# joshua16266261/self-play-ai

Hardware: NVIDIA B200
Metric: MCTS simulations/sec (whole box) Connect4 @800 sims/move (higher is better)
Workload: dtype bf16

## Files before the change

self-play-ai_b200/csrc/evaluator_umma.cu:

```cuda
#include <cuda_bf16.h>

#include <cstring>
#include <mutex>

#include "evaluator_umma.cuh"
#include "umma_ptx.cuh"

namespace spb {
namespace umma {

template <class G>
struct Geo {
  static constexpr int W8 = (G::COLS == 7) ? 8 : 4;
  static constexpr int RP = G::ROWS + 1;
  static constexpr int BS = W8 * RP;
  static constexpr int NT = 4;
  static constexpr int NB = (NT * 128) / BS;
  static constexpr int LEAD = 16;
  static constexpr int Q = LEAD + NT * 128 + 16;
  static constexpr int P = G::ROWS * G::COLS;
  static constexpr int APAD = (G::A <= 8) ? 8 : 16;
};

constexpr int N_LAYERS = 10;
constexpr int HEAD_N = 48;
constexpr int SLOT_BYTES = 8192;
constexpr int N_SLOTS = 9;

__host__ __device__ constexpr int layer_n(int l) { return l == 9 ? HEAD_N : 64; }
__host__ __device__ constexpr int layer_kchunks(int l) { return l == 0 ? 2 : 8; }
__host__ __device__ constexpr int layer_tap_bytes(int l) { return layer_kchunks(l) * layer_n(l) * 16; }
__host__ __device__ constexpr size_t layer_offset(int l) {
  return l == 0 ? 0 : (size_t)9 * 2048 + (size_t)(l - 1) * 9 * SLOT_BYTES;
}
constexpr size_t OFF_BIAS = (size_t)9 * 2048 + (size_t)8 * 9 * SLOT_BYTES + (size_t)9 * 6144;
constexpr size_t OFF_WP = OFF_BIAS + (size_t)N_LAYERS * 64 * 4;
template <class G> __host__ __device__ constexpr size_t off_wv() { return OFF_WP + (size_t)G::A * Geo<G>::P * 32 * 4; }
template <class G> __host__ __device__ constexpr size_t off_fcb() { return off_wv<G>() + (size_t)Geo<G>::P * 8 * 4; }
template <class G> __host__ __device__ constexpr size_t image_bytes() { return off_fcb<G>() + 32 * 4; }

static inline uint16_t f2bf(float f) {
  uint32_t u;
  std::memcpy(&u, &f, 4);
  if ((u & 0x7F800000u) == 0x7F800000u) return (uint16_t)(u >> 16);
  u += 0x7FFFu + ((u >> 16) & 1u);
  return (uint16_t)(u >> 16);
}

template <class G>
static void pack_t(const HostNet& net, std::vector<uint8_t>* out) {
  using Ge = Geo<G>;
  out->assign(image_bytes<G>(), 0);
  uint8_t* img = out->data();
  for (int tap = 0; tap < 9; ++tap) {
    const HostNet::Conv& cv = net.conv[0];
    uint16_t* blk = reinterpret_cast<uint16_t*>(img + layer_offset(0) + (size_t)tap * layer_tap_bytes(0));
    for (int n = 0; n < 64; ++n)
      for (int k = 0; k < 16 && k < cv.ic; ++k)
        blk[((size_t)(k / 8) * 64 + n) * 8 + (k % 8)] = f2bf(cv.w[((size_t)n * cv.ic + k) * 9 + tap]);
  }
  for (int l = 1; l < N_LAYERS; ++l) {
    const int N = layer_n(l), KC = layer_kchunks(l);
    const int n_real = l == 9 ? NET_POLICY_CH + NET_VALUE_CH : 64;
    for (int ky = 0; ky < 3; ++ky) {
      uint16_t* blk = reinterpret_cast<uint16_t*>(img + layer_offset(l) + (size_t)ky * 3 * layer_tap_bytes(l));
      for (int n = 0; n < n_real; ++n) {
        const HostNet::Conv& cv = l < 9 ? net.conv[l] : (n < NET_POLICY_CH ? net.conv[9] : net.conv[10]);
        const int oc = (l == 9 && n >= NET_POLICY_CH) ? n - NET_POLICY_CH : n;
        for (int k = 0; k < KC * 8 && k < cv.ic; ++k) {
          const float* w9 = &cv.w[((size_t)oc * cv.ic + k) * 9 + ky * 3];
          uint16_t* row = blk + ((size_t)(k / 8) * 3 * N) * 8 + (k % 8);
          row[(size_t)n * 8] = f2bf(w9[1]);
          row[(size_t)(N + n) * 8] = f2bf(w9[2]);
          row[(size_t)(2 * N + n) * 8] = f2bf(w9[0]);
        }
      }
    }
  }
  float* bias = reinterpret_cast<float*>(img + OFF_BIAS);
  for (int l = 0; l < 9; ++l)
    for (int n = 0; n < 64; ++n) bias[l * 64 + n] = net.conv[l].b[n];
  for (int n = 0; n < NET_POLICY_CH; ++n) bias[9 * 64 + n] = net.conv[9].b[n];
  for (int n = 0; n < NET_VALUE_CH; ++n) bias[9 * 64 + NET_POLICY_CH + n] = net.conv[10].b[n];
  float* wp = reinterpret_cast<float*>(img + OFF_WP);
  for (int a = 0; a < G::A; ++a)
    for (int pos = 0; pos < Ge::P; ++pos)
      for (int ch = 0; ch < NET_POLICY_CH; ++ch)
        wp[((size_t)a * Ge::P + pos) * NET_POLICY_CH + ch] = net.pfc_w[(size_t)a * NET_POLICY_CH * Ge::P + (size_t)ch * Ge::P + pos];
  float* wv = reinterpret_cast<float*>(img + off_wv<G>());
  for (int pos = 0; pos < Ge::P; ++pos)
    for (int ch = 0; ch < NET_VALUE_CH; ++ch) wv[pos * 8 + ch] = net.vfc_w[(size_t)ch * Ge::P + pos];
  float* fcb = reinterpret_cast<float*>(img + off_fcb<G>());
  for (int a = 0; a < G::A; ++a) fcb[a] = net.pfc_b[a];
  fcb[16] = net.vfc_b[0];
}

void pack_weights(const HostNet& net, std::vector<uint8_t>* out) {
  if (net.game == SPB_GAME_CONNECT4) pack_t<Connect4>(net, out);
  else pack_t<TicTacToe>(net, out);
}

template <int W8, int Q, int KSTEPS, int NP>
__device__ __forceinline__ void issue_tile_triple(bool issuer, uint32_t a_lo_tile, uint32_t b_lo_base, uint32_t d_tmem,
                                                  bool first_tile, bool last_tile, uint32_t w_par, uint32_t bar_base,
                                                  uint32_t mid_bar, uint32_t mid_par) {
  constexpr uint32_t DESC_HI = (128u >> 4) | (1u << 14);
  constexpr uint32_t IDESC = make_idesc(NP);
#pragma unroll
  for (int ky = 0; ky < 3; ++ky) {
    const int shift = (ky - 1) * W8;
    if (ky == 2 && mid_bar) {
      mbar_wait(mid_bar, mid_par);
      tc_fence_after();
    }
    if (first_tile) {
      mbar_wait(bar_base + (uint32_t)ky * 8u, w_par);
      tc_fence_after();
    }
    if (issuer) {
#pragma unroll
      for (int kk = 0; kk < KSTEPS; ++kk) {
        const uint32_t a_lo = a_lo_tile + (uint32_t)(shift + kk * 2 * Q);
        const uint32_t b_lo = (b_lo_base + (uint32_t)(3 * ky) * (SLOT_BYTES >> 4) + (uint32_t)(kk * 2 * NP)) | ((uint32_t)NP << 16);
        umma_f16(d_tmem, ((uint64_t)DESC_HI << 32) | a_lo, ((uint64_t)DESC_HI << 32) | b_lo, IDESC, (ky | kk) != 0);
      }
      if (last_tile) umma_commit(bar_base + (uint32_t)(N_SLOTS + ky) * 8u);
    }
    __syncwarp();
  }
}

template <int W8, int Q>
__device__ __forceinline__ void issue_tile_stem(bool issuer, uint32_t a_lo_tile, uint32_t b_lo_base, uint32_t d_tmem, bool first_tile,
                                                bool last_tile, uint32_t w_par, uint32_t bar_base) {
  constexpr uint32_t DESC_HI = (128u >> 4) | (1u << 14);
  constexpr uint32_t IDESC = make_idesc(64);
#pragma unroll
  for (int ky = 0; ky < 3; ++ky) {
    if (first_tile) {
      mbar_wait(bar_base + (uint32_t)ky * 8u, w_par);
      tc_fence_after();
    }
    if (issuer) {
#pragma unroll
      for (int kx = 0; kx < 3; ++kx) {
        const uint32_t a_lo = a_lo_tile + (uint32_t)((ky - 1) * W8 + (kx - 1));
        const uint32_t b_lo = (b_lo_base + (uint32_t)(3 * ky) * (SLOT_BYTES >> 4) + (uint32_t)kx * (2048u >> 4)) | (64u << 16);
        umma_f16(d_tmem, ((uint64_t)DESC_HI << 32) | a_lo, ((uint64_t)DESC_HI << 32) | b_lo, IDESC, (ky | kx) != 0);
      }
      if (last_tile) umma_commit(bar_base + (uint32_t)(N_SLOTS + ky) * 8u);
    }
    __syncwarp();
  }
}

template <class G>
struct Smem {
  using Ge = Geo<G>;
  static constexpr int ACT_BYTES = 8 * Ge::Q * 16;
  static constexpr int OFF_ACT0 = 0;
  static constexpr int OFF_ACT1 = ACT_BYTES;
  static constexpr int OFF_W = 2 * ACT_BYTES;
  static constexpr int OFF_BIAS = OFF_W + N_SLOTS * SLOT_BYTES;
  static constexpr int OFF_LOGITS = OFF_BIAS + (N_LAYERS * 64 + 32) * 4;
  static constexpr int OFF_PART = OFF_LOGITS + Ge::NB * 16 * 4;
  static constexpr int OFF_STATES = OFF_PART + 8 * Ge::NB * 8 * 4;
  static constexpr int OFF_SLOTS = OFF_STATES + 2 * Ge::NB * 16;
  static constexpr int OFF_BARS = (OFF_SLOTS + 2 * Ge::NB * 4 + 15) & ~15;
  static constexpr int N_BARS = 2 * N_SLOTS + 4 + 2 * Ge::NT + 1 + 3 + 2;
  static constexpr int OFF_TMEM = OFF_BARS + N_BARS * 8;
  static constexpr int OFF_NB = OFF_TMEM + 16;
  static constexpr int TOTAL = OFF_NB + 32;
};
static_assert(Geo<Connect4>::NB <= 32 && Geo<TicTacToe>::NB <= 32, "one stager lane / one publishing lane per board");

static_assert(Smem<Connect4>::TOTAL <= 232448 && Smem<TicTacToe>::TOTAL <= 232448, "shared memory plan exceeds 227 KB");
constexpr int PRODUCER_WARP = 0, MMA_WARP = 1, STAGER_WARP = 2, SPARE_WARP = 3;
constexpr int EPI_WARP0 = 4, N_EPI_WARPS = 8;
constexpr int THREADS = 32 * (EPI_WARP0 + N_EPI_WARPS);
template <class G> struct RingCfg { static constexpr int TREE_WARPS = 4, REGS_LAUNCH = 128, REGS_LIGHT = 72, REGS_TREE = 96, REGS_EPILOGUE = 168; };
template <class G> constexpr int threads_ring() { return THREADS + 32 * RingCfg<G>::TREE_WARPS; }
template <class G> constexpr bool ring_budget_ok() {
  return 128 * RingCfg<G>::REGS_LIGHT + 256 * RingCfg<G>::REGS_EPILOGUE + 32 * RingCfg<G>::TREE_WARPS * RingCfg<G>::REGS_TREE <= threads_ring<G>() * RingCfg<G>::REGS_LAUNCH &&
         threads_ring<G>() * RingCfg<G>::REGS_LAUNCH <= 65536;
}
static_assert(ring_budget_ok<Connect4>() && ring_budget_ok<TicTacToe>(), "setmaxnreg budget exceeds the CTA's launch allocation");
constexpr uint32_t CLAIM_GRACE_NS = 4000;

struct EvalWork {
  const PState* states;
  const uint32_t* list;
  const uint32_t* count_dev;
  uint32_t max_n;
  float* out;
  int stride;
  float* logits_out;
};

#ifdef SPB_TRACE
__device__ unsigned long long g_trace[4][512];
#define TRACE_B0 (RING ? 300u : 0u)
#define TRACE(k, b, l, t) do { if (blockIdx.x == 0 && (b) >= TRACE_B0 && (b) < TRACE_B0 + 12u) g_trace[k][((((b) - TRACE_B0) * 10 + (l)) * 4 + (t))] = clock64(); } while (0)
__device__ unsigned long long g_trace_stager[16][4];
__device__ unsigned long long g_eval_times[64][4];
__device__ unsigned int g_eval_idx = 0;
__device__ __forceinline__ unsigned long long gtimer() { unsigned long long t; asm volatile("mov.u64 %0, %%globaltimer;" : "=l"(t)); return t; }
#define TRACE_ST(b, i) do { if (blockIdx.x == 0 && lane == 0 && (b) >= TRACE_B0 && (b) < TRACE_B0 + 12u) g_trace_stager[(b) - TRACE_B0][i] = clock64(); } while (0)
#define TRACE2(i) do { if (blockIdx.x == 0 && bb == TRACE_B0 && lane == 0) g_trace[3][480 + (warp == EPI_WARP0 ? 0 : 8) + (i)] = clock64(); } while (0)
#define TRACE3(i) do { if (blockIdx.x == 0 && bb == TRACE_B0 + 2u && l == 4 && t == 1 && lane == 0 && (warp == EPI_WARP0 || warp == EPI_WARP0 + 4)) g_trace[3][496 + (warp == EPI_WARP0 ? 0 : 8) + (i)] = clock64(); } while (0)
#else
#define TRACE3(i) ((void)0)
#define TRACE2(i) ((void)0)
#define TRACE(k, b, l, t) ((void)0)
#define TRACE_ST(b, i) ((void)0)
#endif

template <class G, bool RING>
__global__ void __launch_bounds__(RING ? threads_ring<G>() : THREADS, 1)
k_eval_umma(const uint8_t* __restrict__ image, const EvalWork W, const Trees T, const AsyncCtl C) {
  using Ge = Geo<G>;
  using Sm = Smem<G>;
  extern __shared__ __align__(1024) uint8_t smem[];
  const PState* __restrict__ states = RING ? T.leaf_state : W.states;
  const uint32_t* __restrict__ list = W.list;
  float* __restrict__ out = RING ? T.eval_out : W.out;
  const int stride = RING ? G::EVAL_STRIDE : W.stride;
  float* __restrict__ logits_out = RING ? nullptr : W.logits_out;
#ifdef SPB_TRACE
  const unsigned long long tr_entry = gtimer();
#endif
  asm volatile("griddepcontrol.launch_dependents;");
  const int tid = threadIdx.x, warp = tid >> 5, lane = tid & 31;
  const uint32_t s_base = smem_u32(smem);
  const uint32_t bar_base = s_base + Sm::OFF_BARS;
  auto bar_w_full = [&](int s) { return bar_base + (uint32_t)s * 8u; };
  auto bar_w_empty = [&](int s) { return bar_base + (uint32_t)(N_SLOTS + s) * 8u; };
  constexpr uint32_t BAR0 = 2 * N_SLOTS;
  auto bar_acc_full = [&](uint32_t set) { return bar_base + (BAR0 + set) * 8u; };
  auto bar_acc_drained = [&](uint32_t set) { return bar_base + (BAR0 + 2u + set) * 8u; };
  auto bar_act_ready = [&](int t) { return bar_base + (BAR0 + 4u + (uint32_t)t) * 8u; };
  auto bar_stage_ready = [&](int t) { return bar_base + (BAR0 + 4u + (uint32_t)Ge::NT + (uint32_t)t) * 8u; };
  const uint32_t bar_act0_free = bar_base + (BAR0 + 4u + 2u * (uint32_t)Ge::NT) * 8u;
  auto bar_batch = [&](uint32_t bb) { return bar_base + (BAR0 + 5u + 2u * (uint32_t)Ge::NT + (bb & 1u)) * 8u; };
  const uint32_t bar_claim_go = bar_base + (BAR0 + 7u + 2u * (uint32_t)Ge::NT) * 8u;
  const uint32_t bar_out_ready = bar_base + (BAR0 + 8u + 2u * (uint32_t)Ge::NT) * 8u;
  const uint32_t bar_out_free = bar_base + (BAR0 + 9u + 2u * (uint32_t)Ge::NT) * 8u;
  uint32_t* tmem_slot = reinterpret_cast<uint32_t*>(smem + Sm::OFF_TMEM);
  volatile uint32_t* s_nb = reinterpret_cast<volatile uint32_t*>(smem + Sm::OFF_NB);

  {
    uint4 z = make_uint4(0, 0, 0, 0);
    uint4* p = reinterpret_cast<uint4*>(smem);
    for (int i = tid; i < 2 * Sm::ACT_BYTES / 16; i += (int)blockDim.x) p[i] = z;
    const float* gb = reinterpret_cast<const float*>(image + OFF_BIAS);
    float* sb = reinterpret_cast<float*>(smem + Sm::OFF_BIAS);
    for (int i = tid; i < N_LAYERS * 64; i += (int)blockDim.x) sb[i] = gb[i];
    if (tid < 32) sb[N_LAYERS * 64 + tid] = reinterpret_cast<const float*>(image + off_fcb<G>())[tid];
  }
  if (tid == 0) {
    for (int s = 0; s < N_SLOTS; ++s) { mbar_init(bar_w_full(s), 1); mbar_init(bar_w_empty(s), 1); }
    for (uint32_t set = 0; set < 2; ++set) { mbar_init(bar_acc_full(set), 1); mbar_init(bar_acc_drained(set), N_EPI_WARPS); }
    for (int t = 0; t < Ge::NT; ++t) { mbar_init(bar_act_ready(t), N_EPI_WARPS); mbar_init(bar_stage_ready(t), 32); }
    mbar_init(bar_act0_free, 1);
    mbar_init(bar_batch(0), 1); mbar_init(bar_batch(1), 1); mbar_init(bar_claim_go, 1);
    mbar_init(bar_out_ready, 1); mbar_init(bar_out_free, 1);
    asm volatile("fence.mbarrier_init.release.cluster;" ::: "memory");
  }
  if (warp == MMA_WARP) tmem_alloc(smem_u32(tmem_slot), 512);
  fence_async_smem();
  tc_fence_before();
  __syncthreads();
  tc_fence_after();
  const uint32_t tmem_base = *tmem_slot;

  asm volatile("griddepcontrol.wait;" ::: "memory");
#ifdef SPB_TRACE
  const unsigned long long tr_wait = gtimer();
#endif
  const uint32_t n_total = RING ? 0u : min(__ldcg(W.count_dev), W.max_n);
  const uint32_t cta = blockIdx.x, ncta = gridDim.x;
  const uint32_t my_begin = (uint32_t)(((uint64_t)n_total * cta) / ncta);
  const uint32_t my_end = (uint32_t)(((uint64_t)n_total * (cta + 1)) / ncta);
  auto wait_batch = [&](uint32_t bb) -> uint32_t {
    mbar_wait(bar_batch(bb), (bb >> 1) & 1u);
    return s_nb[bb & 3u];
  };

#define SPB_REGS_LIGHT() do { if (RING) asm volatile("setmaxnreg.dec.sync.aligned.u32 %0;" ::"n"(RingCfg<G>::REGS_LIGHT)); } while (0)
#define SPB_REGS_TREE() do { if (RING) asm volatile("setmaxnreg.dec.sync.aligned.u32 %0;" ::"n"(RingCfg<G>::REGS_TREE)); } while (0)
#define SPB_REGS_EPILOGUE() do { if (RING) asm volatile("setmaxnreg.inc.sync.aligned.u32 %0;" ::"n"(RingCfg<G>::REGS_EPILOGUE)); } while (0)

  if (warp == PRODUCER_WARP) {
    SPB_REGS_LIGHT();
    if (lane == 0) {
      uint32_t use = 0;
      for (uint32_t b = 0; wait_batch(b) != 0u; ++b) {
        for (int l = 0; l < N_LAYERS; ++l) {
          const uint32_t bytes = (uint32_t)layer_tap_bytes(l);
          const uint8_t* src = image + layer_offset(l);
          for (int g = 0; g < 3; ++g) {
            if (use > 0) mbar_wait(bar_w_empty(g), (use - 1) & 1u);
            mbar_expect_tx(bar_w_full(g), 3 * bytes);
            bulk_g2s(s_base + Sm::OFF_W + (uint32_t)(3 * g) * SLOT_BYTES, src + (size_t)(3 * g) * bytes, 3 * bytes, bar_w_full(g));
          }
          ++use;
        }
      }
    }
  } else if (warp == MMA_WARP) {
    SPB_REGS_LIGHT();
    {
      const bool issuer = elect_one();
      const uint32_t b_lo_base = ((s_base + Sm::OFF_W) >> 4);
      uint32_t use = 0;
      uint32_t act_par = 0;
      uint32_t stage_par = 0;
      uint32_t g = 0;
      for (uint32_t b = 0;; ++b) {
        const uint32_t nb = wait_batch(b);
        if (nb == 0u) break;
        const int nt = (int)((nb * Ge::BS + 127) / 128);
        for (int l = 0; l < N_LAYERS; ++l) {
          if (RING && l == 7 && issuer) mbar_arrive(bar_claim_go);
          const uint32_t in_buf = s_base + ((l == 0 || (l >= 2 && (l & 1) == 0)) ? Sm::OFF_ACT0 : Sm::OFF_ACT1);
          const uint32_t a_lo_base = ((in_buf >> 4) + Ge::LEAD) | ((uint32_t)Ge::Q << 16);
          const uint32_t cur_par = (l == 0) ? stage_par : act_par;
          if (l == 0) stage_par ^= (1u << nt) - 1u; else act_par ^= (1u << nt) - 1u;
          for (int t = 0; t < nt; ++t, ++g) {
            uint32_t mid_bar = 0, mid_par = 0;
            if (l == 0) {
              const int wt = min(t + 1, nt - 1);
              mbar_wait(bar_stage_ready(wt), (cur_par >> wt) & 1u);
            } else {
              if (t == 0) mbar_wait(bar_act_ready(0), cur_par & 1u);
              if (t + 1 < nt) { mid_bar = bar_act_ready(t + 1); mid_par = (cur_par >> (t + 1)) & 1u; }
            }
            const uint32_t set = g & 1u, u = g >> 1;
            if (u > 0u) mbar_wait(bar_acc_drained(set), (u - 1u) & 1u);
            tc_fence_after();
            if (lane == 0) TRACE(0, b, l, t);
            const uint32_t a_lo_tile = a_lo_base + (uint32_t)t * 128u;
            const uint32_t d_tmem = tmem_base + set * 256u;
            const bool first = (t == 0), last = (t == nt - 1);
            if (l == 0)
              issue_tile_stem<Ge::W8, Ge::Q>(issuer, a_lo_tile, b_lo_base, d_tmem, first, last, use & 1u, bar_base);
            else if (l < 9)
              issue_tile_triple<Ge::W8, Ge::Q, 4, 192>(issuer, a_lo_tile, b_lo_base, d_tmem, first, last, use & 1u, bar_base, mid_bar, mid_par);
            else
              issue_tile_triple<Ge::W8, Ge::Q, 4, 3 * HEAD_N>(issuer, a_lo_tile, b_lo_base, d_tmem, first, last, use & 1u, bar_base, mid_bar, mid_par);
            if (issuer) {
              umma_commit(bar_acc_full(set));
              if (l == 8 && last) umma_commit(bar_act0_free);
            }
            __syncwarp();
            if (lane == 0) TRACE(1, b, l, t);
          }
          ++use;
        }
      }
    }
  } else if (warp == STAGER_WARP) {
    SPB_REGS_LIGHT();
    PState* s_states = reinterpret_cast<PState*>(smem + Sm::OFF_STATES);
    uint32_t* s_slots = reinterpret_cast<uint32_t*>(smem + Sm::OFF_SLOTS);
    Spin sp;
    if (RING) sp.init(C, *C.n_active);
    unsigned long long st_batches = 0, st_boards = 0, st_wait = 0;
    LeafClaimer lc;
    for (uint32_t bb = 0;; ++bb) {
      uint32_t nb = 0;
      PState st_mine = PState{};
      uint32_t slot_mine = 0;
      if (RING) {
        if (bb > 0) mbar_wait_backoff<64>(bar_claim_go, (bb - 1) & 1u);
        const unsigned long long tw0 = gtime_ns();
        TRACE_ST(bb, 0);
        nb = claim_batch(C, lc, ncta, (uint32_t)Ge::NB, CLAIM_GRACE_NS, sp, lane, &slot_mine);
        if (nb) { st_wait += gtime_ns() - tw0; ++st_batches; st_boards += nb; }
        TRACE_ST(bb, 1);
      } else {
        const uint32_t b0 = my_begin + bb * Ge::NB;
        nb = b0 < my_end ? min((uint32_t)Ge::NB, my_end - b0) : 0u;
        if ((uint32_t)lane < nb) slot_mine = list ? __ldcg(list + b0 + lane) : (b0 + lane);
      }
      if (lane == 0) {
        s_nb[bb & 3u] = nb;
        mbar_arrive(bar_batch(bb));
      }
      if (nb == 0u) {
        if (RING && lane == 0) {
          atomicAdd(&C.stats[ASTAT_BATCHES], st_batches);
          atomicAdd(&C.stats[ASTAT_BOARDS], st_boards);
          atomicAdd(&C.stats[ASTAT_CLAIM_WAIT_NS], st_wait);
          atomicAdd(&C.stats[ASTAT_EVAL_CTAS], 1ull);
        }
        break;
      }
      const int nt = (int)((nb * Ge::BS + 127) / 128);
      if ((uint32_t)lane < nb) {
        const ulonglong2 raw = __ldcg(reinterpret_cast<const ulonglong2*>(states + slot_mine));
        st_mine.x = raw.x; st_mine.o = raw.y;
      }
      if (bb > 0) mbar_wait_backoff<64>(bar_act0_free, (bb - 1) & 1u);
      TRACE_ST(bb, 2);
      PState* st_buf = s_states + (bb & 1u) * Ge::NB;
      if ((uint32_t)lane < nb) { s_slots[(bb & 1u) * Ge::NB + lane] = slot_mine; st_buf[lane] = st_mine; }
      __syncwarp();
      for (int t = 0; t < nt; ++t) {
#pragma unroll
        for (int q = 0; q < 4; ++q) {
          const int m = t * 128 + q * 32 + lane;
          const int bi = m / Ge::BS, rem = m % Ge::BS, r = rem / Ge::W8, c = rem % Ge::W8;
          uint4 v0 = make_uint4(0, 0, 0, 0);
          if ((uint32_t)bi < nb && r < G::ROWS && c < G::COLS) {
            const PState st = st_buf[bi];
            const float e0 = G::encode_cell(st, 0, r, c), e1 = G::encode_cell(st, 1, r, c), e2 = G::encode_cell(st, 2, r, c);
            v0.x = pack_bf16x2(e0, e1);
            v0.y = pack_bf16x2(e2, 0.0f);
          }
          *reinterpret_cast<uint4*>(smem + Sm::OFF_ACT0 + (size_t)(Ge::LEAD + m) * 16) = v0;
          *reinterpret_cast<uint4*>(smem + Sm::OFF_ACT0 + (size_t)Ge::Q * 16 + (size_t)(Ge::LEAD + m) * 16) = make_uint4(0, 0, 0, 0);
        }
        fence_async_smem();
        mbar_arrive(bar_stage_ready(t));
      }
      TRACE_ST(bb, 3);
    }
  } else if (warp >= EPI_WARP0 && warp < EPI_WARP0 + N_EPI_WARPS) {
    SPB_REGS_EPILOGUE();
    const int et = tid - 32 * EPI_WARP0;
    const int quad = warp & 3;
    const int half = (warp - EPI_WARP0) >> 2;
    const int row_in_tile = quad * 32 + lane;
    const float* s_bias = reinterpret_cast<const float*>(smem + Sm::OFF_BIAS);
    float* s_logits = reinterpret_cast<float*>(smem + Sm::OFF_LOGITS);
    uint32_t* s_slots = reinterpret_cast<uint32_t*>(smem + Sm::OFF_SLOTS);
    const float* g_wp = reinterpret_cast<const float*>(image + OFF_WP);
    const float* g_wv = reinterpret_cast<const float*>(image + off_wv<G>());
    uint32_t eg = 0;

    auto conv_epilogue = [&](uint32_t bb, int l, int t_begin = 0, int t_end = Ge::NT) {
      const uint32_t nb = s_nb[bb & 3u];
      const int nt = min((int)((nb * Ge::BS + 127) / 128), t_end);
      const bool in0 = (l == 0 || (l >= 2 && (l & 1) == 0));
      uint8_t* dst_buf = smem + (in0 ? Sm::OFF_ACT1 : Sm::OFF_ACT0);
      const bool has_skip = (l >= 2 && (l & 1) == 0);
      const bool stash_skip = (l & 1) == 0 && l <= 6;
      float bias_r[32];
#pragma unroll
      for (int q = 0; q < 8; ++q) {
        const float4 bv = *reinterpret_cast<const float4*>(s_bias + l * 64 + half * 32 + q * 4);
        bias_r[4 * q] = bv.x; bias_r[4 * q + 1] = bv.y; bias_r[4 * q + 2] = bv.z; bias_r[4 * q + 3] = bv.w;
      }
      for (int t = t_begin; t < nt; ++t, ++eg) {
        const int m = t * 128 + row_in_tile;
        const int bi = m / Ge::BS, rem = m % Ge::BS, r = rem / Ge::W8, c = rem % Ge::W8;
        const bool valid = (uint32_t)bi < nb && r < G::ROWS && c < G::COLS;
        uint8_t* drow = dst_buf + (size_t)(half * 4) * Ge::Q * 16 + (size_t)(Ge::LEAD + m) * 16;
        const uint32_t set = eg & 1u;
        TRACE3(0);
        mbar_wait(bar_acc_full(set), (eg >> 1) & 1u);
        tc_fence_after();
        if (et == 0) TRACE(2, bb, l, t);
        TRACE3(1);
        const uint32_t taddr = tmem_base + ((uint32_t)(quad * 32) << 16) + set * 256u + (uint32_t)half * 32u;
        uint32_t a[32], e[32], f[32];
        tmem_ld16(taddr, a);
        tmem_ld16(taddr + 16u, a + 16);
        if (l != 0) {
          tmem_ld16(taddr + 64u, e);
          tmem_ld16(taddr + 80u, e + 16);
          tmem_ld16(taddr + 128u, f);
          tmem_ld16(taddr + 144u, f + 16);
        }
        tmem_ld_wait();
        tc_fence_before();
        __syncwarp();
        if (lane == 0) mbar_arrive(bar_acc_drained(set));
        TRACE3(2);
        float v[32];
#pragma unroll
        for (int q = 0; q < 32; q += 2) {
          if (l == 0) { v[q] = __uint_as_float(a[q]); v[q + 1] = __uint_as_float(a[q + 1]); continue; }
          const float e0 = __uint_as_float(__shfl_down_sync(0xffffffffu, e[q], 1)), e1 = __uint_as_float(__shfl_down_sync(0xffffffffu, e[q + 1], 1));
          const float f0 = __uint_as_float(__shfl_up_sync(0xffffffffu, f[q], 1)), f1 = __uint_as_float(__shfl_up_sync(0xffffffffu, f[q + 1], 1));
          v[q] = __uint_as_float(a[q]); v[q + 1] = __uint_as_float(a[q + 1]);
          add2(v[q], v[q + 1], e0, e1);
          if (lane != 0) add2(v[q], v[q + 1], f0, f1);
        }
        TRACE3(3);
        const uint32_t skaddr = tmem_base + ((uint32_t)(quad * 32) << 16) + ((t & 1) ? 448u : 192u) + (uint32_t)(t >> 1) * 32u + (uint32_t)half * 16u;
        uint32_t sk[16];
        if (has_skip) tmem_ld16(skaddr, sk);
#pragma unroll
        for (int q = 0; q < 32; q += 2) add2(v[q], v[q + 1], bias_r[q], bias_r[q + 1]);
        if (has_skip) {
          tmem_ld_wait();
#pragma unroll
          for (int q = 0; q < 16; ++q) add2(v[2 * q], v[2 * q + 1], bf_lo(sk[q]), bf_hi(sk[q]));
        }
        uint32_t o[16];
#pragma unroll
        for (int q = 0; q < 16; ++q) o[q] = valid ? pack_relu_bf16x2(v[2 * q], v[2 * q + 1]) : 0u;
#pragma unroll
        for (int j = 0; j < 4; ++j)
          *reinterpret_cast<uint4*>(drow + (size_t)j * Ge::Q * 16) = make_uint4(o[4 * j], o[4 * j + 1], o[4 * j + 2], o[4 * j + 3]);
        if (stash_skip) { tmem_st16(skaddr, o); tmem_st_wait(); }
        TRACE3(4);
        fence_async_smem();
        __syncwarp();
        if (lane == 0) mbar_arrive(bar_act_ready(t));
        TRACE3(5);
        if (et == 0) TRACE(3, bb, l, t);
      }
    };

    auto head_epilogue = [&](uint32_t bb) {
      const uint32_t nb = s_nb[bb & 3u];
      const int nt = (int)((nb * Ge::BS + 127) / 128);
      const float* bias = s_bias + 9 * 64;
      for (int t = 0; t < nt; ++t, ++eg) {
        const int m = t * 128 + row_in_tile;
        const int bi = m / Ge::BS, rem = m % Ge::BS, r = rem / Ge::W8, c = rem % Ge::W8;
        const bool valid = (uint32_t)bi < nb && r < G::ROWS && c < G::COLS;
        const uint32_t set = eg & 1u;
        mbar_wait(bar_acc_full(set), (eg >> 1) & 1u);
        tc_fence_after();
        if (et == 0) TRACE(2, bb, 9, t);
        const uint32_t taddr = tmem_base + ((uint32_t)(quad * 32) << 16) + set * 256u;
        uint32_t a[16], av[4], e[16], ev[4], f[16], fv[4];
        tmem_ld16(taddr + (uint32_t)half * 16u, a);
        tmem_ld16(taddr + (uint32_t)HEAD_N + (uint32_t)half * 16u, e);
        tmem_ld16(taddr + 2u * (uint32_t)HEAD_N + (uint32_t)half * 16u, f);
        if (half == 1) { tmem_ld4(taddr + 32u, av); tmem_ld4(taddr + (uint32_t)HEAD_N + 32u, ev); tmem_ld4(taddr + 2u * (uint32_t)HEAD_N + 32u, fv); }
        tmem_ld_wait();
        tc_fence_before();
        __syncwarp();
        if (lane == 0) mbar_arrive(bar_acc_drained(set));
#pragma unroll
        for (int q = 0; q < 16; ++q) {
          const float e1 = __uint_as_float(__shfl_down_sync(0xffffffffu, e[q], 1));
          const float f1 = __uint_as_float(__shfl_up_sync(0xffffffffu, f[q], 1));
          float v = __uint_as_float(a[q]) + e1;
          if (lane != 0) v += f1;
          a[q] = __float_as_uint(v);
        }
        if (half == 1) {
#pragma unroll
          for (int q = 0; q < 3; ++q) {
            const float e1 = __uint_as_float(__shfl_down_sync(0xffffffffu, ev[q], 1));
            const float f1 = __uint_as_float(__shfl_up_sync(0xffffffffu, fv[q], 1));
            av[q] = __float_as_uint((__uint_as_float(av[q]) + e1) + (lane == 0 ? 0.0f : f1));
          }
        }
        if (valid) {
          uint8_t* prow = smem + Sm::OFF_ACT0 + (size_t)(Ge::LEAD + m) * 16;
#pragma unroll
          for (int j = 0; j < 2; ++j) {
            uint4 o;
            const float* bj = bias + half * 16 + j * 8;
            o.x = pack_bf16x2(fmaxf(__uint_as_float(a[j * 8 + 0]) + bj[0], 0.f), fmaxf(__uint_as_float(a[j * 8 + 1]) + bj[1], 0.f));
            o.y = pack_bf16x2(fmaxf(__uint_as_float(a[j * 8 + 2]) + bj[2], 0.f), fmaxf(__uint_as_float(a[j * 8 + 3]) + bj[3], 0.f));
            o.z = pack_bf16x2(fmaxf(__uint_as_float(a[j * 8 + 4]) + bj[4], 0.f), fmaxf(__uint_as_float(a[j * 8 + 5]) + bj[5], 0.f));
            o.w = pack_bf16x2(fmaxf(__uint_as_float(a[j * 8 + 6]) + bj[6], 0.f), fmaxf(__uint_as_float(a[j * 8 + 7]) + bj[7], 0.f));
            *reinterpret_cast<uint4*>(prow + (size_t)(2 + half * 2 + j) * Ge::Q * 16) = o;
          }
          if (half == 1) {
            uint4 o = make_uint4(0, 0, 0, 0);
            o.x = pack_bf16x2(fmaxf(__uint_as_float(av[0]) + bias[32], 0.f), fmaxf(__uint_as_float(av[1]) + bias[33], 0.f));
            o.y = pack_bf16x2(fmaxf(__uint_as_float(av[2]) + bias[34], 0.f), 0.f);
            *reinterpret_cast<uint4*>(prow + (size_t)6 * Ge::Q * 16) = o;
          }
        }
        if (et == 0) TRACE(3, bb, 9, t);
      }
    };

    constexpr int LH_P = Ge::P;
    constexpr int NOUT = G::A + 1;
    const bool is_pol = et < 4 * LH_P, is_val = !is_pol && et < 5 * LH_P;
    const int pos = is_pol ? (et % LH_P) : (is_val ? et - 4 * LH_P : 0);
    const int c4 = is_pol ? (et / LH_P) : 4;
    auto load_head_weights = [&](float (&w)[8][8], int og) {
#pragma unroll
      for (int s = 0; s < 8; ++s) {
        const int o = og + s;
#pragma unroll
        for (int j = 0; j < 8; ++j) w[s][j] = 0.0f;
        const float* src = nullptr;
        if (is_pol && o < G::A) src = g_wp + ((size_t)o * LH_P + pos) * NET_POLICY_CH + c4 * 8;
        if (is_val && o == G::A) src = g_wv + pos * 8;
        if (src) {
          const float4 w0 = __ldg(reinterpret_cast<const float4*>(src)), w1 = __ldg(reinterpret_cast<const float4*>(src) + 1);
          w[s][0] = w0.x; w[s][1] = w0.y; w[s][2] = w0.z; w[s][3] = w0.w;
          w[s][4] = w1.x; w[s][5] = w1.y; w[s][6] = w1.z; w[s][7] = w1.w;
        }
      }
    };
    auto heads_partials = [&](uint32_t bb, float (&w)[8][8], uint32_t bi_begin = 0, uint32_t bi_end = Ge::NB) {
      const uint32_t nb = s_nb[bb & 3u];
      const uint32_t bend = min(nb, bi_end);
      float* s_part = reinterpret_cast<float*>(smem + Sm::OFF_PART);
      const int we = warp - EPI_WARP0;
      const uint32_t roff = (uint32_t)((is_pol || is_val ? (2 + c4) * Ge::Q * 16 : 0) + ((pos / G::COLS) * Ge::W8 + (pos % G::COLS)) * 16);
      TRACE2(0);
      {
        TRACE2(1);
        const bool b4 = lane & 16, b3 = lane & 8, b2 = lane & 4;
        uint4 vn[3];
#pragma unroll
        for (int k = 0; k < 3; ++k)
          vn[k] = *reinterpret_cast<const uint4*>(smem + Sm::OFF_ACT0 + (size_t)(Ge::LEAD + min(bi_begin + (uint32_t)k, nb - 1u) * Ge::BS) * 16 + roff);
        for (uint32_t bi0 = bi_begin; bi0 < bend; bi0 += 3) {
          float sres[3];
          uint4 v[3];
#pragma unroll
          for (int k = 0; k < 3; ++k) {
            v[k] = vn[k];
            vn[k] = *reinterpret_cast<const uint4*>(smem + Sm::OFF_ACT0 + (size_t)(Ge::LEAD + min(bi0 + 3u + (uint32_t)k, nb - 1u) * Ge::BS) * 16 + roff);
          }
          float q[3][4], r2[3][2];
#pragma unroll
          for (int k = 0; k < 3; ++k) {
            const float x0 = bf_lo(v[k].x), x1 = bf_hi(v[k].x), x2 = bf_lo(v[k].y), x3 = bf_hi(v[k].y);
            const float x4 = bf_lo(v[k].z), x5 = bf_hi(v[k].z), x6 = bf_lo(v[k].w), x7 = bf_hi(v[k].w);
            float p[8];
#pragma unroll
            for (int s = 0; s < 8; ++s) {
              float a = x0 * w[s][0];
              a = fmaf(x1, w[s][1], a); a = fmaf(x2, w[s][2], a); a = fmaf(x3, w[s][3], a);
              a = fmaf(x4, w[s][4], a); a = fmaf(x5, w[s][5], a); a = fmaf(x6, w[s][6], a); a = fmaf(x7, w[s][7], a);
              p[s] = a;
            }
#pragma unroll
            for (int i = 0; i < 4; ++i) q[k][i] = (b4 ? p[i + 4] : p[i]) + __shfl_xor_sync(0xffffffffu, b4 ? p[i] : p[i + 4], 16);
          }
#pragma unroll
          for (int k = 0; k < 3; ++k) {
#pragma unroll
            for (int i = 0; i < 2; ++i) r2[k][i] = (b3 ? q[k][i + 2] : q[k][i]) + __shfl_xor_sync(0xffffffffu, b3 ? q[k][i] : q[k][i + 2], 8);
          }
#pragma unroll
          for (int k = 0; k < 3; ++k) sres[k] = (b2 ? r2[k][1] : r2[k][0]) + __shfl_xor_sync(0xffffffffu, b2 ? r2[k][0] : r2[k][1], 4);
#pragma unroll
          for (int k = 0; k < 3; ++k) sres[k] += __shfl_xor_sync(0xffffffffu, sres[k], 2);
#pragma unroll
          for (int k = 0; k < 3; ++k) sres[k] += __shfl_xor_sync(0xffffffffu, sres[k], 1);
          if ((lane & 3) == 0) {
#pragma unroll
            for (int k = 0; k < 3; ++k)
              if (bi0 + (uint32_t)k < nb) s_part[((size_t)we * Ge::NB + bi0 + k) * 8 + (lane >> 2)] = sres[k];
          }
        }
        TRACE2(2);
      }
    };
    auto heads_reduce = [&](uint32_t bb, int og) {
      const uint32_t nb = s_nb[bb & 3u];
      const float* s_part = reinterpret_cast<const float*>(smem + Sm::OFF_PART);
      epi_bar_sync();
      if (og == 0 && bb > 0) mbar_wait(bar_out_free, (bb - 1) & 1u);
      for (int i = et; i < (int)nb * 8; i += 256) {
        const int bi = i >> 3, sl = i & 7, o = og + sl;
        if (o < NOUT) {
          float acc = 0.0f;
#pragma unroll
          for (int wv_ = 0; wv_ < 8; ++wv_) acc += s_part[((size_t)wv_ * Ge::NB + bi) * 8 + sl];
          s_logits[bi * 16 + (o == G::A ? 15 : o)] = acc;
        }
      }
      epi_bar_sync();
      TRACE2(3);
    };
    auto heads_softmax = [&](uint32_t bb) {
      const uint32_t nb = s_nb[bb & 3u];
      constexpr int LG = G::A <= 7 ? 8 : 16;
      const float* fcb = s_bias + N_LAYERS * 64;
      const int a = et % LG;
      for (uint32_t bi = (uint32_t)(et / LG); bi < ((nb + 256 / LG - 1) / (256 / LG)) * (256 / LG); bi += 256 / LG) {
        const bool live = bi < nb;
        const float raw = live ? s_logits[bi * 16 + (a == LG - 1 ? 15 : a)] : 0.0f;
        const float lg = (a < G::A) ? raw + fcb[a] : -INFINITY;
        float mx = lg;
#pragma unroll
        for (int o = LG / 2; o >= 1; o >>= 1) mx = fmaxf(mx, __shfl_xor_sync(0xffffffffu, mx, o));
        const float ex = (a < G::A) ? expf(lg - mx) : 0.0f;
        float sum = 0.0f;
#pragma unroll
        for (int k = 0; k < G::A; ++k) sum += __shfl_sync(0xffffffffu, ex, (lane & ~(LG - 1)) + k);
        if (live) {
          if (a < G::A) s_logits[bi * 16 + a] = ex / sum;
          else if (a == LG - 1) s_logits[bi * 16 + 15] = tanhf(raw + fcb[16]);
          if (logits_out && a < G::A) logits_out[(size_t)s_slots[(bb & 1u) * Ge::NB + bi] * G::A + a] = lg;
        }
      }
      TRACE2(4);
      epi_bar_sync();
      if (et == 0) mbar_arrive(bar_out_ready);
      TRACE2(5);
    };
    auto linear_heads = [&](uint32_t bb, float (&w_first)[8][8]) {
      heads_partials(bb, w_first);
      heads_reduce(bb, 0);
      for (int og = 8; og < NOUT; og += 8) {
        float w[8][8];
        load_head_weights(w, og);
        heads_partials(bb, w);
        heads_reduce(bb, og);
      }
      heads_softmax(bb);
    };

    constexpr uint32_t NOT_YET = 0xFFFFFFFFu;
    uint32_t nb_cur = wait_batch(0);
    if (nb_cur != 0u) conv_epilogue(0, 0);
    bool l1_done = false;
    for (uint32_t b = 0; nb_cur != 0u; ++b) {
      for (int l = l1_done ? 2 : 1; l < 9; ++l) conv_epilogue(b, l);
      l1_done = false;
      head_epilogue(b);
      if (et == 0) s_nb[4] = mbar_test(bar_batch(b + 1), ((b + 1) >> 1) & 1u) ? s_nb[(b + 1) & 3u] : NOT_YET;
      epi_bar_sync();
      uint32_t nb_next = s_nb[4];
      float w_heads[8][8];
      if (nb_next != NOT_YET) {
        load_head_weights(w_heads, 0);
        if (nb_next != 0u) conv_epilogue(b + 1, 0);
        if (NOUT <= 8 && nb_next != 0u) {
          heads_partials(b, w_heads);
          epi_bar_sync();
          conv_epilogue(b + 1, 1);
          l1_done = true;
          heads_reduce(b, 0);
          heads_softmax(b);
        } else {
          linear_heads(b, w_heads);
        }
      } else {
        load_head_weights(w_heads, 0);
        linear_heads(b, w_heads);
        nb_next = wait_batch(b + 1);
        if (nb_next != 0u) conv_epilogue(b + 1, 0);
      }
      nb_cur = nb_next;
    }
  }

  if (RING && warp >= EPI_WARP0 + N_EPI_WARPS) {
    SPB_REGS_TREE();
    tree_worker<G>(T, C, lane);
  } else if (warp == SPARE_WARP) {
    SPB_REGS_LIGHT();
    const float* s_logits = reinterpret_cast<const float*>(smem + Sm::OFF_LOGITS);
    const uint32_t* s_slots = reinterpret_cast<const uint32_t*>(smem + Sm::OFF_SLOTS);
    for (uint32_t b = 0;; ++b) {
      const uint32_t nb = wait_batch(b);
      if (nb == 0u) break;
      mbar_wait(bar_out_ready, b & 1u);
      uint32_t slot = 0;
      float rec[G::A + 1];
      if ((uint32_t)lane < nb) {
        slot = s_slots[(b & 1u) * Ge::NB + lane];
#pragma unroll
        for (int a = 0; a < G::A; ++a) rec[a] = s_logits[lane * 16 + a];
        rec[G::A] = s_logits[lane * 16 + 15];
      }
      __syncwarp();
      if (lane == 0) mbar_arrive(bar_out_free);
      if ((uint32_t)lane < nb) {
        float* o = out + (size_t)slot * stride;
#pragma unroll
        for (int a = 0; a <= G::A; ++a) o[a] = rec[a];
      }
      if (RING) ring_push_warp(C.ready, nb, slot, lane);
    }
  }

  tc_fence_before();
  __syncthreads();
  if (warp == MMA_WARP) { tc_fence_after(); tmem_dealloc(tmem_base, 512); }
#ifdef SPB_TRACE
  if (blockIdx.x == 0 && tid == 0) {
    const unsigned int i = g_eval_idx++ & 63u;
    g_eval_times[i][0] = tr_entry; g_eval_times[i][1] = tr_wait; g_eval_times[i][2] = gtimer();
  }
#endif
}

template <class G, bool RING>
static cudaError_t prepare(int* sm_count_out) {
  static std::mutex mu;
  static int sm_counts[64] = {};
  int dev = 0;
  cudaError_t e = cudaGetDevice(&dev);
  if (e != cudaSuccess) return e;
  if (dev < 0 || dev >= 64) return cudaErrorInvalidDevice;
  std::lock_guard<std::mutex> lock(mu);
  if (sm_counts[dev] == 0) {
    int n = 0;
    e = cudaDeviceGetAttribute(&n, cudaDevAttrMultiProcessorCount, dev);
    if (e == cudaSuccess) e = cudaFuncSetAttribute(k_eval_umma<G, RING>, cudaFuncAttributeMaxDynamicSharedMemorySize, Smem<G>::TOTAL);
    if (e != cudaSuccess) return e;
    sm_counts[dev] = n;
  }
  *sm_count_out = sm_counts[dev];
  return cudaSuccess;
}

template <class G>
static cudaError_t launch_t(const Evaluator::DevNet& net, const PState* states, const uint32_t* list, const uint32_t* count_dev,
                            uint32_t max_n, float* out, int stride, float* logits_out, cudaStream_t stream, bool overlap) {
  int sm_count = 0;
  cudaError_t e = prepare<G, false>(&sm_count);
  if (e != cudaSuccess) return e;
  const unsigned grid = (unsigned)std::max(1, std::min<int>(sm_count, (int)max_n));
  cudaLaunchConfig_t cfg = {};
  cfg.gridDim = dim3(grid);
  cfg.blockDim = dim3(THREADS);
  cfg.dynamicSmemBytes = Smem<G>::TOTAL;
  cfg.stream = stream;
  cudaLaunchAttribute attr[1];
  attr[0].id = cudaLaunchAttributeProgrammaticStreamSerialization;
  attr[0].val.programmaticStreamSerializationAllowed = overlap ? 1 : 0;
  cfg.attrs = attr;
  cfg.numAttrs = 1;
  EvalWork W{states, list, count_dev, max_n, out, stride, logits_out};
  return cudaLaunchKernelEx(&cfg, k_eval_umma<G, false>, reinterpret_cast<const uint8_t*>(net.w_umma), W, Trees{}, AsyncCtl{});
}

template <class G>
static cudaError_t launch_ring_t(const Evaluator::DevNet& net, const Trees& T, const AsyncCtl& C, cudaStream_t stream) {
  int sm_count = 0;
  cudaError_t e = prepare<G, true>(&sm_count);
  if (e != cudaSuccess) return e;
  const unsigned grid = (unsigned)std::max(1, std::min<int>(sm_count, (int)T.G));
  k_eval_umma<G, true><<<grid, threads_ring<G>(), Smem<G>::TOTAL, stream>>>(reinterpret_cast<const uint8_t*>(net.w_umma), EvalWork{}, T, C);
  return cudaGetLastError();
}

#ifdef SPB_TRACE
extern "C" int spb_debug_eval_times_v2(unsigned long long* out) {
  unsigned int z = 0;
  int rc = (int)cudaMemcpyFromSymbol(out, g_eval_times, sizeof(unsigned long long) * 64 * 4);
  rc |= (int)cudaMemcpyToSymbol(g_eval_idx, &z, sizeof z);
  return rc;
}
extern "C" int spb_debug_trace_stager(unsigned long long* out) { return (int)cudaMemcpyFromSymbol(out, g_trace_stager, sizeof(unsigned long long) * 16 * 4); }
extern "C" int spb_debug_trace_v2(unsigned long long* out, int reset) {
  int rc = (int)cudaMemcpyFromSymbol(out, g_trace, sizeof(unsigned long long) * 4 * 512);
  if (reset) { static unsigned long long z[4 * 512]; rc |= (int)cudaMemcpyToSymbol(g_trace, z, sizeof z); }
  return rc;
}
#endif

cudaError_t launch(const Evaluator::DevNet& net, int game, const PState* states, const uint32_t* list, const uint32_t* count_dev,
                   uint32_t max_n, float* out, int stride, float* logits_out, cudaStream_t stream, bool overlap) {
  if (game == SPB_GAME_CONNECT4) return launch_t<Connect4>(net, states, list, count_dev, max_n, out, stride, logits_out, stream, overlap);
  return launch_t<TicTacToe>(net, states, list, count_dev, max_n, out, stride, logits_out, stream, overlap);
}

cudaError_t launch_ring(const Evaluator::DevNet& net, int game, const Trees& T, const AsyncCtl& C, cudaStream_t stream) {
  if (game == SPB_GAME_CONNECT4) return launch_ring_t<Connect4>(net, T, C, stream);
  return launch_ring_t<TicTacToe>(net, T, C, stream);
}

}
}
```

self-play-ai_b200/csrc/umma_ptx.cuh:

```cuda
#pragma once
#include <cuda_bf16.h>
#include <cstdint>

namespace spb {
namespace umma {

__device__ __forceinline__ uint32_t smem_u32(const void* p) { return (uint32_t)__cvta_generic_to_shared(p); }
__device__ __forceinline__ void mbar_init(uint32_t bar, uint32_t count) { asm volatile("mbarrier.init.shared::cta.b64 [%0], %1;" ::"r"(bar), "r"(count)); }
__device__ __forceinline__ void mbar_wait(uint32_t bar, uint32_t parity) {
  uint32_t ok;
  do {
#ifdef SPB_MBAR_HINT
    asm volatile("{\n.reg .pred p;\nmbarrier.try_wait.parity.shared::cta.b64 p, [%1], %2, %3;\nselp.u32 %0, 1, 0, p;\n}"
                 : "=r"(ok) : "r"(bar), "r"(parity), "r"((uint32_t)SPB_MBAR_HINT) : "memory");
#else
    asm volatile("{\n.reg .pred p;\nmbarrier.try_wait.parity.shared::cta.b64 p, [%1], %2;\nselp.u32 %0, 1, 0, p;\n}"
                 : "=r"(ok) : "r"(bar), "r"(parity) : "memory");
#endif
  } while (!ok);
}
__device__ __forceinline__ void mbar_wait_sleep(uint32_t bar, uint32_t parity) {
  uint32_t ok;
  for (;;) {
    asm volatile("{\n.reg .pred p;\nmbarrier.try_wait.parity.shared::cta.b64 p, [%1], %2;\nselp.u32 %0, 1, 0, p;\n}"
                 : "=r"(ok) : "r"(bar), "r"(parity) : "memory");
    if (ok) break;
    __nanosleep(200);
  }
}
template <int NS>
__device__ __forceinline__ void mbar_wait_backoff(uint32_t bar, uint32_t parity) {
  uint32_t ok;
  for (;;) {
    asm volatile("{\n.reg .pred p;\nmbarrier.try_wait.parity.shared::cta.b64 p, [%1], %2;\nselp.u32 %0, 1, 0, p;\n}"
                 : "=r"(ok) : "r"(bar), "r"(parity) : "memory");
    if (ok) break;
    if (NS > 0) __nanosleep(NS);
  }
}
__device__ __forceinline__ bool mbar_test(uint32_t bar, uint32_t parity) {
  uint32_t ok;
  asm volatile("{\n.reg .pred p;\nmbarrier.test_wait.parity.shared::cta.b64 p, [%1], %2;\nselp.u32 %0, 1, 0, p;\n}"
               : "=r"(ok) : "r"(bar), "r"(parity) : "memory");
  return ok != 0;
}
__device__ __forceinline__ void mbar_arrive(uint32_t bar) { asm volatile("mbarrier.arrive.shared::cta.b64 _, [%0];" ::"r"(bar) : "memory"); }
__device__ __forceinline__ void mbar_expect_tx(uint32_t bar, uint32_t bytes) { asm volatile("mbarrier.arrive.expect_tx.shared::cta.b64 _, [%0], %1;" ::"r"(bar), "r"(bytes) : "memory"); }
__device__ __forceinline__ void bulk_g2s(uint32_t dst, const void* src, uint32_t bytes, uint32_t bar) {
  asm volatile("cp.async.bulk.shared::cluster.global.mbarrier::complete_tx::bytes [%0], [%1], %2, [%3];" ::"r"(dst), "l"(src), "r"(bytes), "r"(bar) : "memory");
}
__device__ __forceinline__ void tmem_alloc(uint32_t dst_smem, uint32_t ncols) {
  asm volatile("tcgen05.alloc.cta_group::1.sync.aligned.shared::cta.b32 [%0], %1;" ::"r"(dst_smem), "r"(ncols) : "memory");
  asm volatile("tcgen05.relinquish_alloc_permit.cta_group::1.sync.aligned;" ::: "memory");
}
__device__ __forceinline__ void tmem_dealloc(uint32_t taddr, uint32_t ncols) { asm volatile("tcgen05.dealloc.cta_group::1.sync.aligned.b32 %0, %1;" ::"r"(taddr), "r"(ncols) : "memory"); }
__device__ __forceinline__ void umma_f16(uint32_t d_tmem, uint64_t adesc, uint64_t bdesc, uint32_t idesc, uint32_t accumulate) {
  asm volatile("{\n.reg .pred p;\nsetp.ne.b32 p, %4, 0;\ntcgen05.mma.cta_group::1.kind::f16 [%0], %1, %2, %3, p;\n}"
               ::"r"(d_tmem), "l"(adesc), "l"(bdesc), "r"(idesc), "r"(accumulate) : "memory");
}
__device__ __forceinline__ void umma_commit(uint32_t bar) { asm volatile("tcgen05.commit.cta_group::1.mbarrier::arrive::one.shared::cluster.b64 [%0];" ::"r"(bar) : "memory"); }
__device__ __forceinline__ void tc_fence_before() { asm volatile("tcgen05.fence::before_thread_sync;" ::: "memory"); }
__device__ __forceinline__ void tc_fence_after() { asm volatile("tcgen05.fence::after_thread_sync;" ::: "memory"); }
__device__ __forceinline__ void fence_async_smem() { asm volatile("fence.proxy.async.shared::cta;" ::: "memory"); }
__device__ __forceinline__ bool elect_one() {
  uint32_t pred;
  asm volatile("{\n.reg .pred P1;\nelect.sync _|P1, 0xffffffff;\nselp.u32 %0, 1, 0, P1;\n}" : "=r"(pred));
  return pred != 0;
}
__device__ __forceinline__ void epi_bar_sync() { asm volatile("bar.sync 1, 256;" ::: "memory"); }

__device__ __forceinline__ void tmem_ld16(uint32_t taddr, uint32_t* r) {
  asm volatile("tcgen05.ld.sync.aligned.32x32b.x16.b32 {%0,%1,%2,%3,%4,%5,%6,%7,%8,%9,%10,%11,%12,%13,%14,%15}, [%16];"
               : "=r"(r[0]), "=r"(r[1]), "=r"(r[2]), "=r"(r[3]), "=r"(r[4]), "=r"(r[5]), "=r"(r[6]), "=r"(r[7]), "=r"(r[8]), "=r"(r[9]),
                 "=r"(r[10]), "=r"(r[11]), "=r"(r[12]), "=r"(r[13]), "=r"(r[14]), "=r"(r[15])
               : "r"(taddr));
}
__device__ __forceinline__ void tmem_ld4(uint32_t taddr, uint32_t* r) {
  asm volatile("tcgen05.ld.sync.aligned.32x32b.x4.b32 {%0,%1,%2,%3}, [%4];" : "=r"(r[0]), "=r"(r[1]), "=r"(r[2]), "=r"(r[3]) : "r"(taddr));
}
__device__ __forceinline__ void tmem_st16(uint32_t taddr, const uint32_t* r) {
  asm volatile("tcgen05.st.sync.aligned.32x32b.x16.b32 [%0], {%1,%2,%3,%4,%5,%6,%7,%8,%9,%10,%11,%12,%13,%14,%15,%16};"
               ::"r"(taddr), "r"(r[0]), "r"(r[1]), "r"(r[2]), "r"(r[3]), "r"(r[4]), "r"(r[5]), "r"(r[6]), "r"(r[7]), "r"(r[8]), "r"(r[9]),
                 "r"(r[10]), "r"(r[11]), "r"(r[12]), "r"(r[13]), "r"(r[14]), "r"(r[15]) : "memory");
}
__device__ __forceinline__ void tmem_st_wait() { asm volatile("tcgen05.wait::st.sync.aligned;" ::: "memory"); }
__device__ __forceinline__ void tmem_ld_wait() { asm volatile("tcgen05.wait::ld.sync.aligned;" ::: "memory"); }

__device__ __forceinline__ uint64_t make_desc(uint32_t addr, uint32_t lbo, uint32_t sbo) {
  return (uint64_t)((addr >> 4) & 0x3FFFu) | ((uint64_t)((lbo >> 4) & 0x3FFFu) << 16) | ((uint64_t)((sbo >> 4) & 0x3FFFu) << 32) |
         ((uint64_t)1 << 46);
}
__host__ __device__ constexpr uint32_t make_idesc(int N) {
  return (1u << 4) | (1u << 7) | (1u << 10) | ((uint32_t)(N >> 3) << 17) | ((uint32_t)(128 >> 4) << 24);
}

__device__ __forceinline__ uint32_t pack_bf16x2(float lo, float hi) {
  __nv_bfloat162 v = __floats2bfloat162_rn(lo, hi);
  return *reinterpret_cast<uint32_t*>(&v);
}
__device__ __forceinline__ void add2(float& x0, float& x1, float y0, float y1) {
  uint64_t x, y;
  asm("mov.b64 %0, {%1, %2};" : "=l"(x) : "f"(x0), "f"(x1));
  asm("mov.b64 %0, {%1, %2};" : "=l"(y) : "f"(y0), "f"(y1));
  asm("add.rn.f32x2 %0, %0, %1;" : "+l"(x) : "l"(y));
  asm("mov.b64 {%0, %1}, %2;" : "=f"(x0), "=f"(x1) : "l"(x));
}
__device__ __forceinline__ uint32_t pack_relu_bf16x2(float lo, float hi) {
  uint32_t d;
  asm("cvt.rn.relu.bf16x2.f32 %0, %1, %2;" : "=r"(d) : "f"(hi), "f"(lo));
  return d;
}
__device__ __forceinline__ float bf_lo(uint32_t u) { return __uint_as_float(u << 16); }
__device__ __forceinline__ float bf_hi(uint32_t u) { return __uint_as_float(u & 0xFFFF0000u); }

}
}
```

Before: 45.82 million.

## Fuse policy/value FC into head epilogue with per-tile partial sums

The head conv epilogue now computes the policy and value linear layers directly from its TMEM accumulators. Each thread applies register-held or shared-memory-staged weights and reduces partials with warp shuffles into a per-board shared buffer. The spare warp finishes the cross-group sum, softmax and tanh, which removes the activation write-back to shared memory, the separate partials, reduce and softmax phases, and several named barriers. The head layer also uses smaller tiles aligned to whole boards, and the MMA warp waits only on the activation tiles each head tile needs. This costs more registers in the epilogue warps, extra shared memory for the weights, and the overlap of the head with the next batch's early layers is dropped.

Result: no change. 45.72 million (median of 6 runs) (-0.2%).

```diff
diff --git a/self-play-ai_b200/csrc/evaluator_umma.cu b/self-play-ai_b200/csrc/evaluator_umma.cu
--- a/self-play-ai_b200/csrc/evaluator_umma.cu
+++ b/self-play-ai_b200/csrc/evaluator_umma.cu
@@ -19,7 +19,9 @@
   static constexpr int LEAD = 16;
   static constexpr int Q = LEAD + NT * 128 + 16;
   static constexpr int P = G::ROWS * G::COLS;
-  static constexpr int APAD = (G::A <= 8) ? 8 : 16;
+  static constexpr int HB = 128 / BS;
+  static constexpr int HS = HB * BS;
+  static constexpr int HG = BS / 8;
 };
 
 constexpr int N_LAYERS = 10;
@@ -86,7 +88,7 @@
   for (int a = 0; a < G::A; ++a)
     for (int pos = 0; pos < Ge::P; ++pos)
       for (int ch = 0; ch < NET_POLICY_CH; ++ch)
-        wp[((size_t)a * Ge::P + pos) * NET_POLICY_CH + ch] = net.pfc_w[(size_t)a * NET_POLICY_CH * Ge::P + (size_t)ch * Ge::P + pos];
+        wp[(((size_t)a * 8 + ch / 4) * Ge::P + pos) * 4 + ch % 4] = net.pfc_w[(size_t)a * NET_POLICY_CH * Ge::P + (size_t)ch * Ge::P + pos];
   float* wv = reinterpret_cast<float*>(img + off_wv<G>());
   for (int pos = 0; pos < Ge::P; ++pos)
     for (int ch = 0; ch < NET_VALUE_CH; ++ch) wv[pos * 8 + ch] = net.vfc_w[(size_t)ch * Ge::P + pos];
@@ -152,6 +154,12 @@
     }
     __syncwarp();
   }
+}
+
+__device__ __forceinline__ float4 ldg_f4_here(const float* p) {
+  float4 v;
+  asm volatile("ld.global.nc.v4.f32 {%0,%1,%2,%3}, [%4];" : "=f"(v.x), "=f"(v.y), "=f"(v.z), "=f"(v.w) : "l"(p));
+  return v;
 }
 
 template <class G>
@@ -162,9 +170,13 @@
   static constexpr int OFF_ACT1 = ACT_BYTES;
   static constexpr int OFF_W = 2 * ACT_BYTES;
   static constexpr int OFF_BIAS = OFF_W + N_SLOTS * SLOT_BYTES;
-  static constexpr int OFF_LOGITS = OFF_BIAS + (N_LAYERS * 64 + 32) * 4;
-  static constexpr int OFF_PART = OFF_LOGITS + Ge::NB * 16 * 4;
-  static constexpr int OFF_STATES = OFF_PART + 8 * Ge::NB * 8 * 4;
+  static constexpr int OREG = G::A <= 7 ? 6 : 4;
+  static constexpr int NOUTP = (G::A + 1 + 7) & ~7;
+  static constexpr int OFF_WPS = OFF_BIAS + (N_LAYERS * 64 + 32) * 4;
+  static constexpr int OFF_WVS = OFF_WPS + (G::A - OREG) * 2 * 16 * Ge::P * 4;
+  static constexpr int OFF_HPART = OFF_WVS + Ge::P * 16;
+  static constexpr int HPART_BOARD = Ge::HG * 2 * NOUTP + 1;
+  static constexpr int OFF_STATES = (OFF_HPART + Ge::NB * HPART_BOARD * 4 + 15) & ~15;
   static constexpr int OFF_SLOTS = OFF_STATES + 2 * Ge::NB * 16;
   static constexpr int OFF_BARS = (OFF_SLOTS + 2 * Ge::NB * 4 + 15) & ~15;
   static constexpr int N_BARS = 2 * N_SLOTS + 4 + 2 * Ge::NT + 1 + 3 + 2;
@@ -198,19 +210,17 @@
 };
 
 #ifdef SPB_TRACE
-__device__ unsigned long long g_trace[4][512];
+__device__ unsigned long long g_trace[4][1024];
 #define TRACE_B0 (RING ? 300u : 0u)
-#define TRACE(k, b, l, t) do { if (blockIdx.x == 0 && (b) >= TRACE_B0 && (b) < TRACE_B0 + 12u) g_trace[k][((((b) - TRACE_B0) * 10 + (l)) * 4 + (t))] = clock64(); } while (0)
+#define TRACE(k, b, l, t) do { if (blockIdx.x == 0 && (b) >= TRACE_B0 && (b) < TRACE_B0 + 12u) g_trace[k][((((b) - TRACE_B0) * 10 + (l)) * 8 + (t))] = clock64(); } while (0)
 __device__ unsigned long long g_trace_stager[16][4];
 __device__ unsigned long long g_eval_times[64][4];
 __device__ unsigned int g_eval_idx = 0;
 __device__ __forceinline__ unsigned long long gtimer() { unsigned long long t; asm volatile("mov.u64 %0, %%globaltimer;" : "=l"(t)); return t; }
 #define TRACE_ST(b, i) do { if (blockIdx.x == 0 && lane == 0 && (b) >= TRACE_B0 && (b) < TRACE_B0 + 12u) g_trace_stager[(b) - TRACE_B0][i] = clock64(); } while (0)
-#define TRACE2(i) do { if (blockIdx.x == 0 && bb == TRACE_B0 && lane == 0) g_trace[3][480 + (warp == EPI_WARP0 ? 0 : 8) + (i)] = clock64(); } while (0)
-#define TRACE3(i) do { if (blockIdx.x == 0 && bb == TRACE_B0 + 2u && l == 4 && t == 1 && lane == 0 && (warp == EPI_WARP0 || warp == EPI_WARP0 + 4)) g_trace[3][496 + (warp == EPI_WARP0 ? 0 : 8) + (i)] = clock64(); } while (0)
+#define TRACE3(i) do { if (blockIdx.x == 0 && bb == TRACE_B0 + 2u && l == 4 && t == 1 && lane == 0 && (warp == EPI_WARP0 || warp == EPI_WARP0 + 4)) g_trace[3][992 + (warp == EPI_WARP0 ? 0 : 8) + (i)] = clock64(); } while (0)
 #else
 #define TRACE3(i) ((void)0)
-#define TRACE2(i) ((void)0)
 #define TRACE(k, b, l, t) ((void)0)
 #define TRACE_ST(b, i) ((void)0)
 #endif
@@ -256,6 +266,11 @@
     float* sb = reinterpret_cast<float*>(smem + Sm::OFF_BIAS);
     for (int i = tid; i < N_LAYERS * 64; i += (int)blockDim.x) sb[i] = gb[i];
     if (tid < 32) sb[N_LAYERS * 64 + tid] = reinterpret_cast<const float*>(image + off_fcb<G>())[tid];
+    const float4* gw = reinterpret_cast<const float4*>(image + OFF_WP) + Sm::OREG * 8 * Ge::P;
+    float4* sw = reinterpret_cast<float4*>(smem + Sm::OFF_WPS);
+    for (int i = tid; i < (G::A - Sm::OREG) * 8 * Ge::P; i += (int)blockDim.x) sw[i] = gw[i];
+    for (int i = tid; i < Ge::P; i += (int)blockDim.x)
+      reinterpret_cast<float4*>(smem + Sm::OFF_WVS)[i] = reinterpret_cast<const float4*>(image + off_wv<G>())[2 * i];
   }
   if (tid == 0) {
     for (int s = 0; s < N_SLOTS; ++s) { mbar_init(bar_w_full(s), 1); mbar_init(bar_w_empty(s), 1); }
@@ -263,7 +278,7 @@
     for (int t = 0; t < Ge::NT; ++t) { mbar_init(bar_act_ready(t), N_EPI_WARPS); mbar_init(bar_stage_ready(t), 32); }
     mbar_init(bar_act0_free, 1);
     mbar_init(bar_batch(0), 1); mbar_init(bar_batch(1), 1); mbar_init(bar_claim_go, 1);
-    mbar_init(bar_out_ready, 1); mbar_init(bar_out_free, 1);
+    mbar_init(bar_out_ready, N_EPI_WARPS); mbar_init(bar_out_free, 1);
     asm volatile("fence.mbarrier_init.release.cluster;" ::: "memory");
   }
   if (warp == MMA_WARP) tmem_alloc(smem_u32(tmem_slot), 512);
@@ -320,28 +335,32 @@
         const uint32_t nb = wait_batch(b);
         if (nb == 0u) break;
         const int nt = (int)((nb * Ge::BS + 127) / 128);
+        const int nht = (int)((nb + Ge::HB - 1) / Ge::HB);
         for (int l = 0; l < N_LAYERS; ++l) {
           if (RING && l == 7 && issuer) mbar_arrive(bar_claim_go);
           const uint32_t in_buf = s_base + ((l == 0 || (l >= 2 && (l & 1) == 0)) ? Sm::OFF_ACT0 : Sm::OFF_ACT1);
           const uint32_t a_lo_base = ((in_buf >> 4) + Ge::LEAD) | ((uint32_t)Ge::Q << 16);
           const uint32_t cur_par = (l == 0) ? stage_par : act_par;
           if (l == 0) stage_par ^= (1u << nt) - 1u; else act_par ^= (1u << nt) - 1u;
-          for (int t = 0; t < nt; ++t, ++g) {
+          const int ntl = l == 9 ? nht : nt, ts = l == 9 ? Ge::HS : 128;
+          int waited = 0;
+          for (int t = 0; t < ntl; ++t, ++g) {
             uint32_t mid_bar = 0, mid_par = 0;
             if (l == 0) {
               const int wt = min(t + 1, nt - 1);
               mbar_wait(bar_stage_ready(wt), (cur_par >> wt) & 1u);
             } else {
-              if (t == 0) mbar_wait(bar_act_ready(0), cur_par & 1u);
-              if (t + 1 < nt) { mid_bar = bar_act_ready(t + 1); mid_par = (cur_par >> (t + 1)) & 1u; }
+              const int need = min((ts * t + 127) / 128, nt - 1), need_mid = min((ts * t + 127 + Ge::W8) / 128, nt - 1);
+              for (; waited <= need; ++waited) mbar_wait(bar_act_ready(waited), (cur_par >> waited) & 1u);
+              if (need_mid >= waited) { mid_bar = bar_act_ready(need_mid); mid_par = (cur_par >> need_mid) & 1u; waited = need_mid + 1; }
             }
             const uint32_t set = g & 1u, u = g >> 1;
             if (u > 0u) mbar_wait(bar_acc_drained(set), (u - 1u) & 1u);
             tc_fence_after();
             if (lane == 0) TRACE(0, b, l, t);
-            const uint32_t a_lo_tile = a_lo_base + (uint32_t)t * 128u;
+            const uint32_t a_lo_tile = a_lo_base + (uint32_t)(t * ts);
             const uint32_t d_tmem = tmem_base + set * 256u;
-            const bool first = (t == 0), last = (t == nt - 1);
+            const bool first = (t == 0), last = (t == ntl - 1);
             if (l == 0)
               issue_tile_stem<Ge::W8, Ge::Q>(issuer, a_lo_tile, b_lo_base, d_tmem, first, last, use & 1u, bar_base);
             else if (l < 9)
@@ -433,10 +452,7 @@
     const int half = (warp - EPI_WARP0) >> 2;
     const int row_in_tile = quad * 32 + lane;
     const float* s_bias = reinterpret_cast<const float*>(smem + Sm::OFF_BIAS);
-    float* s_logits = reinterpret_cast<float*>(smem + Sm::OFF_LOGITS);
-    uint32_t* s_slots = reinterpret_cast<uint32_t*>(smem + Sm::OFF_SLOTS);
     const float* g_wp = reinterpret_cast<const float*>(image + OFF_WP);
-    const float* g_wv = reinterpret_cast<const float*>(image + off_wv<G>());
     uint32_t eg = 0;
 
     auto conv_epilogue = [&](uint32_t bb, int l, int t_begin = 0, int t_end = Ge::NT) {
@@ -516,242 +532,122 @@
     };
 
     auto head_epilogue = [&](uint32_t bb) {
+      constexpr int OREG = Sm::OREG, NOUTP = Sm::NOUTP;
       const uint32_t nb = s_nb[bb & 3u];
-      const int nt = (int)((nb * Ge::BS + 127) / 128);
+      const int nht = (int)((nb + Ge::HB - 1) / Ge::HB);
       const float* bias = s_bias + 9 * 64;
-      for (int t = 0; t < nt; ++t, ++eg) {
-        const int m = t * 128 + row_in_tile;
-        const int bi = m / Ge::BS, rem = m % Ge::BS, r = rem / Ge::W8, c = rem % Ge::W8;
-        const bool valid = (uint32_t)bi < nb && r < G::ROWS && c < G::COLS;
+      const int rem = row_in_tile % Ge::BS, r = rem / Ge::W8, c = rem % Ge::W8, grp = rem >> 3;
+      const bool cell = row_in_tile < Ge::HS && r < G::ROWS && c < G::COLS;
+      const int pos = cell ? r * G::COLS + c : 0;
+      float w[OREG][16];
+#pragma unroll
+      for (int o = 0; o < OREG; ++o) {
+#pragma unroll
+        for (int q = 0; q < 4; ++q) {
+          const float4 v = ldg_f4_here(g_wp + (((size_t)o * 8 + half * 4 + q) * Ge::P + pos) * 4);
+          w[o][4 * q] = v.x; w[o][4 * q + 1] = v.y; w[o][4 * q + 2] = v.z; w[o][4 * q + 3] = v.w;
+        }
+      }
+      const float4* s_wps = reinterpret_cast<const float4*>(smem + Sm::OFF_WPS) + half * 4 * Ge::P + pos;
+      float* s_hpart = reinterpret_cast<float*>(smem + Sm::OFF_HPART);
+      for (int t = 0; t < nht; ++t, ++eg) {
+        const uint32_t bi = (uint32_t)(t * Ge::HB + row_in_tile / Ge::BS);
+        const bool valid = cell && bi < nb;
         const uint32_t set = eg & 1u;
         mbar_wait(bar_acc_full(set), (eg >> 1) & 1u);
         tc_fence_after();
         if (et == 0) TRACE(2, bb, 9, t);
         const uint32_t taddr = tmem_base + ((uint32_t)(quad * 32) << 16) + set * 256u;
-        uint32_t a[16], av[4], e[16], ev[4], f[16], fv[4];
+        uint32_t a[16], av[4], e[16], ev[4];
         tmem_ld16(taddr + (uint32_t)half * 16u, a);
         tmem_ld16(taddr + (uint32_t)HEAD_N + (uint32_t)half * 16u, e);
-        tmem_ld16(taddr + 2u * (uint32_t)HEAD_N + (uint32_t)half * 16u, f);
-        if (half == 1) { tmem_ld4(taddr + 32u, av); tmem_ld4(taddr + (uint32_t)HEAD_N + 32u, ev); tmem_ld4(taddr + 2u * (uint32_t)HEAD_N + 32u, fv); }
+        tmem_ld4(taddr + 32u, av);
+        tmem_ld4(taddr + (uint32_t)HEAD_N + 32u, ev);
+        tmem_ld_wait();
+        float v[20];
+#pragma unroll
+        for (int q = 0; q < 16; q += 2) {
+          v[q] = __uint_as_float(a[q]); v[q + 1] = __uint_as_float(a[q + 1]);
+          add2(v[q], v[q + 1], __uint_as_float(__shfl_down_sync(0xffffffffu, e[q], 1)), __uint_as_float(__shfl_down_sync(0xffffffffu, e[q + 1], 1)));
+        }
+#pragma unroll
+        for (int q = 0; q < 4; q += 2) {
+          v[16 + q] = __uint_as_float(av[q]); v[17 + q] = __uint_as_float(av[q + 1]);
+          add2(v[16 + q], v[17 + q], __uint_as_float(__shfl_down_sync(0xffffffffu, ev[q], 1)), __uint_as_float(__shfl_down_sync(0xffffffffu, ev[q + 1], 1)));
+        }
+        tmem_ld16(taddr + 2u * (uint32_t)HEAD_N + (uint32_t)half * 16u, e);
+        tmem_ld4(taddr + 2u * (uint32_t)HEAD_N + 32u, ev);
         tmem_ld_wait();
         tc_fence_before();
         __syncwarp();
         if (lane == 0) mbar_arrive(bar_acc_drained(set));
-#pragma unroll
-        for (int q = 0; q < 16; ++q) {
-          const float e1 = __uint_as_float(__shfl_down_sync(0xffffffffu, e[q], 1));
-          const float f1 = __uint_as_float(__shfl_up_sync(0xffffffffu, f[q], 1));
-          float v = __uint_as_float(a[q]) + e1;
-          if (lane != 0) v += f1;
-          a[q] = __float_as_uint(v);
-        }
-        if (half == 1) {
-#pragma unroll
-          for (int q = 0; q < 3; ++q) {
-            const float e1 = __uint_as_float(__shfl_down_sync(0xffffffffu, ev[q], 1));
-            const float f1 = __uint_as_float(__shfl_up_sync(0xffffffffu, fv[q], 1));
-            av[q] = __float_as_uint((__uint_as_float(av[q]) + e1) + (lane == 0 ? 0.0f : f1));
+        if (t == 0 && bb > 0) mbar_wait(bar_out_free, (bb - 1) & 1u);
+        uint32_t xp[10];
+#pragma unroll
+        for (int q = 0; q < 20; q += 2) {
+          const uint32_t* fs = q < 16 ? e + q : ev + (q - 16);
+          const float f0 = __uint_as_float(__shfl_up_sync(0xffffffffu, fs[0], 1)), f1 = __uint_as_float(__shfl_up_sync(0xffffffffu, fs[1], 1));
+          if (lane != 0) add2(v[q], v[q + 1], f0, f1);
+          const float4 bq = *reinterpret_cast<const float4*>(bias + (q < 16 ? half * 16 + (q & ~3) : 32 + ((q - 16) & ~3)));
+          add2(v[q], v[q + 1], (q & 2) ? bq.z : bq.x, (q & 2) ? bq.w : bq.y);
+          xp[q / 2] = valid ? pack_relu_bf16x2(v[q], v[q + 1]) : 0u;
+        }
+        auto partial = [&](int o) -> float {
+          float s0 = 0.f, s1 = 0.f;
+          if (o < OREG) {
+#pragma unroll
+            for (int k = 0; k < 8; ++k) fma2(s0, s1, bf_lo(xp[k]), bf_hi(xp[k]), w[o][2 * k], w[o][2 * k + 1]);
+          } else if (o < G::A) {
+#pragma unroll
+            for (int q = 0; q < 4; ++q) {
+              const float4 wq = s_wps[((o - OREG) * 8 + q) * Ge::P];
+              fma2(s0, s1, bf_lo(xp[2 * q]), bf_hi(xp[2 * q]), wq.x, wq.y);
+              fma2(s0, s1, bf_lo(xp[2 * q + 1]), bf_hi(xp[2 * q + 1]), wq.z, wq.w);
+            }
+          } else if (o == G::A) {
+            const float4 wv = reinterpret_cast<const float4*>(smem + Sm::OFF_WVS)[pos];
+            fma2(s0, s1, bf_lo(xp[8]), bf_hi(xp[8]), half == 1 ? wv.x : 0.f, half == 1 ? wv.y : 0.f);
+            s0 = fmaf(bf_lo(xp[9]), half == 1 ? wv.z : 0.f, s0);
           }
-        }
-        if (valid) {
-          uint8_t* prow = smem + Sm::OFF_ACT0 + (size_t)(Ge::LEAD + m) * 16;
-#pragma unroll
-          for (int j = 0; j < 2; ++j) {
-            uint4 o;
-            const float* bj = bias + half * 16 + j * 8;
-            o.x = pack_bf16x2(fmaxf(__uint_as_float(a[j * 8 + 0]) + bj[0], 0.f), fmaxf(__uint_as_float(a[j * 8 + 1]) + bj[1], 0.f));
-            o.y = pack_bf16x2(fmaxf(__uint_as_float(a[j * 8 + 2]) + bj[2], 0.f), fmaxf(__uint_as_float(a[j * 8 + 3]) + bj[3], 0.f));
-            o.z = pack_bf16x2(fmaxf(__uint_as_float(a[j * 8 + 4]) + bj[4], 0.f), fmaxf(__uint_as_float(a[j * 8 + 5]) + bj[5], 0.f));
-            o.w = pack_bf16x2(fmaxf(__uint_as_float(a[j * 8 + 6]) + bj[6], 0.f), fmaxf(__uint_as_float(a[j * 8 + 7]) + bj[7], 0.f));
-            *reinterpret_cast<uint4*>(prow + (size_t)(2 + half * 2 + j) * Ge::Q * 16) = o;
-          }
-          if (half == 1) {
-            uint4 o = make_uint4(0, 0, 0, 0);
-            o.x = pack_bf16x2(fmaxf(__uint_as_float(av[0]) + bias[32], 0.f), fmaxf(__uint_as_float(av[1]) + bias[33], 0.f));
-            o.y = pack_bf16x2(fmaxf(__uint_as_float(av[2]) + bias[34], 0.f), 0.f);
-            *reinterpret_cast<uint4*>(prow + (size_t)6 * Ge::Q * 16) = o;
-          }
+          return s0 + s1;
+        };
+        const bool b2 = lane & 4, b1 = lane & 2, b0 = lane & 1;
+        const bool store = row_in_tile < Ge::HS && bi < nb;
+        float* dst = s_hpart + bi * Sm::HPART_BOARD + (grp * 2 + half) * NOUTP + (lane & 7);
+#pragma unroll
+        for (int k = 0; k < NOUTP / 8; ++k) {
+          float pk[8], q4[4], q2[2];
+#pragma unroll
+          for (int i = 0; i < 8; ++i) pk[i] = partial(8 * k + i);
+#pragma unroll
+          for (int i = 0; i < 4; ++i) q4[i] = (b2 ? pk[i + 4] : pk[i]) + __shfl_xor_sync(0xffffffffu, b2 ? pk[i] : pk[i + 4], 4);
+#pragma unroll
+          for (int i = 0; i < 2; ++i) q2[i] = (b1 ? q4[i + 2] : q4[i]) + __shfl_xor_sync(0xffffffffu, b1 ? q4[i] : q4[i + 2], 2);
+          const float sum = (b0 ? q2[1] : q2[0]) + __shfl_xor_sync(0xffffffffu, b0 ? q2[0] : q2[1], 1);
+          if (store) dst[8 * k] = sum;
         }
         if (et == 0) TRACE(3, bb, 9, t);
       }
+      __syncwarp();
+      if (lane == 0) mbar_arrive(bar_out_ready);
     };
 
-    constexpr int LH_P = Ge::P;
-    constexpr int NOUT = G::A + 1;
-    const bool is_pol = et < 4 * LH_P, is_val = !is_pol && et < 5 * LH_P;
-    const int pos = is_pol ? (et % LH_P) : (is_val ? et - 4 * LH_P : 0);
-    const int c4 = is_pol ? (et / LH_P) : 4;
-    auto load_head_weights = [&](float (&w)[8][8], int og) {
-#pragma unroll
-      for (int s = 0; s < 8; ++s) {
-        const int o = og + s;
-#pragma unroll
-        for (int j = 0; j < 8; ++j) w[s][j] = 0.0f;
-        const float* src = nullptr;
-        if (is_pol && o < G::A) src = g_wp + ((size_t)o * LH_P + pos) * NET_POLICY_CH + c4 * 8;
-        if (is_val && o == G::A) src = g_wv + pos * 8;
-        if (src) {
-          const float4 w0 = __ldg(reinterpret_cast<const float4*>(src)), w1 = __ldg(reinterpret_cast<const float4*>(src) + 1);
-          w[s][0] = w0.x; w[s][1] = w0.y; w[s][2] = w0.z; w[s][3] = w0.w;
-          w[s][4] = w1.x; w[s][5] = w1.y; w[s][6] = w1.z; w[s][7] = w1.w;
-        }
-      }
-    };
-    auto heads_partials = [&](uint32_t bb, float (&w)[8][8], uint32_t bi_begin = 0, uint32_t bi_end = Ge::NB) {
-      const uint32_t nb = s_nb[bb & 3u];
-      const uint32_t bend = min(nb, bi_end);
-      float* s_part = reinterpret_cast<float*>(smem + Sm::OFF_PART);
-      const int we = warp - EPI_WARP0;
-      const uint32_t roff = (uint32_t)((is_pol || is_val ? (2 + c4) * Ge::Q * 16 : 0) + ((pos / G::COLS) * Ge::W8 + (pos % G::COLS)) * 16);
-      TRACE2(0);
-      {
-        TRACE2(1);
-        const bool b4 = lane & 16, b3 = lane & 8, b2 = lane & 4;
-        uint4 vn[3];
-#pragma unroll
-        for (int k = 0; k < 3; ++k)
-          vn[k] = *reinterpret_cast<const uint4*>(smem + Sm::OFF_ACT0 + (size_t)(Ge::LEAD + min(bi_begin + (uint32_t)k, nb - 1u) * Ge::BS) * 16 + roff);
-        for (uint32_t bi0 = bi_begin; bi0 < bend; bi0 += 3) {
-          float sres[3];
-          uint4 v[3];
-#pragma unroll
-          for (int k = 0; k < 3; ++k) {
-            v[k] = vn[k];
-            vn[k] = *reinterpret_cast<const uint4*>(smem + Sm::OFF_ACT0 + (size_t)(Ge::LEAD + min(bi0 + 3u + (uint32_t)k, nb - 1u) * Ge::BS) * 16 + roff);
-          }
-          float q[3][4], r2[3][2];
-#pragma unroll
-          for (int k = 0; k < 3; ++k) {
-            const float x0 = bf_lo(v[k].x), x1 = bf_hi(v[k].x), x2 = bf_lo(v[k].y), x3 = bf_hi(v[k].y);
-            const float x4 = bf_lo(v[k].z), x5 = bf_hi(v[k].z), x6 = bf_lo(v[k].w), x7 = bf_hi(v[k].w);
-            float p[8];
-#pragma unroll
-            for (int s = 0; s < 8; ++s) {
-              float a = x0 * w[s][0];
-              a = fmaf(x1, w[s][1], a); a = fmaf(x2, w[s][2], a); a = fmaf(x3, w[s][3], a);
-              a = fmaf(x4, w[s][4], a); a = fmaf(x5, w[s][5], a); a = fmaf(x6, w[s][6], a); a = fmaf(x7, w[s][7], a);
-              p[s] = a;
-            }
-#pragma unroll
-            for (int i = 0; i < 4; ++i) q[k][i] = (b4 ? p[i + 4] : p[i]) + __shfl_xor_sync(0xffffffffu, b4 ? p[i] : p[i + 4], 16);
-          }
-#pragma unroll
-          for (int k = 0; k < 3; ++k) {
-#pragma unroll
-            for (int i = 0; i < 2; ++i) r2[k][i] = (b3 ? q[k][i + 2] : q[k][i]) + __shfl_xor_sync(0xffffffffu, b3 ? q[k][i] : q[k][i + 2], 8);
-          }
-#pragma unroll
-          for (int k = 0; k < 3; ++k) sres[k] = (b2 ? r2[k][1] : r2[k][0]) + __shfl_xor_sync(0xffffffffu, b2 ? r2[k][0] : r2[k][1], 4);
-#pragma unroll
-          for (int k = 0; k < 3; ++k) sres[k] += __shfl_xor_sync(0xffffffffu, sres[k], 2);
-#pragma unroll
-          for (int k = 0; k < 3; ++k) sres[k] += __shfl_xor_sync(0xffffffffu, sres[k], 1);
-          if ((lane & 3) == 0) {
-#pragma unroll
-            for (int k = 0; k < 3; ++k)
-              if (bi0 + (uint32_t)k < nb) s_part[((size_t)we * Ge::NB + bi0 + k) * 8 + (lane >> 2)] = sres[k];
-          }
-        }
-        TRACE2(2);
-      }
-    };
-    auto heads_reduce = [&](uint32_t bb, int og) {
-      const uint32_t nb = s_nb[bb & 3u];
-      const float* s_part = reinterpret_cast<const float*>(smem + Sm::OFF_PART);
-      epi_bar_sync();
-      if (og == 0 && bb > 0) mbar_wait(bar_out_free, (bb - 1) & 1u);
-      for (int i = et; i < (int)nb * 8; i += 256) {
-        const int bi = i >> 3, sl = i & 7, o = og + sl;
-        if (o < NOUT) {
-          float acc = 0.0f;
-#pragma unroll
-          for (int wv_ = 0; wv_ < 8; ++wv_) acc += s_part[((size_t)wv_ * Ge::NB + bi) * 8 + sl];
-          s_logits[bi * 16 + (o == G::A ? 15 : o)] = acc;
-        }
-      }
-      epi_bar_sync();
-      TRACE2(3);
-    };
-    auto heads_softmax = [&](uint32_t bb) {
-      const uint32_t nb = s_nb[bb & 3u];
-      constexpr int LG = G::A <= 7 ? 8 : 16;
-      const float* fcb = s_bias + N_LAYERS * 64;
-      const int a = et % LG;
-      for (uint32_t bi = (uint32_t)(et / LG); bi < ((nb + 256 / LG - 1) / (256 / LG)) * (256 / LG); bi += 256 / LG) {
-        const bool live = bi < nb;
-        const float raw = live ? s_logits[bi * 16 + (a == LG - 1 ? 15 : a)] : 0.0f;
-        const float lg = (a < G::A) ? raw + fcb[a] : -INFINITY;
-        float mx = lg;
-#pragma unroll
-        for (int o = LG / 2; o >= 1; o >>= 1) mx = fmaxf(mx, __shfl_xor_sync(0xffffffffu, mx, o));
-        const float ex = (a < G::A) ? expf(lg - mx) : 0.0f;
-        float sum = 0.0f;
-#pragma unroll
-        for (int k = 0; k < G::A; ++k) sum += __shfl_sync(0xffffffffu, ex, (lane & ~(LG - 1)) + k);
-        if (live) {
-          if (a < G::A) s_logits[bi * 16 + a] = ex / sum;
-          else if (a == LG - 1) s_logits[bi * 16 + 15] = tanhf(raw + fcb[16]);
-          if (logits_out && a < G::A) logits_out[(size_t)s_slots[(bb & 1u) * Ge::NB + bi] * G::A + a] = lg;
-        }
-      }
-      TRACE2(4);
-      epi_bar_sync();
-      if (et == 0) mbar_arrive(bar_out_ready);
-      TRACE2(5);
-    };
-    auto linear_heads = [&](uint32_t bb, float (&w_first)[8][8]) {
-      heads_partials(bb, w_first);
-      heads_reduce(bb, 0);
-      for (int og = 8; og < NOUT; og += 8) {
-        float w[8][8];
-        load_head_weights(w, og);
-        heads_partials(bb, w);
-        heads_reduce(bb, og);
-      }
-      heads_softmax(bb);
-    };
-
-    constexpr uint32_t NOT_YET = 0xFFFFFFFFu;
     uint32_t nb_cur = wait_batch(0);
     if (nb_cur != 0u) conv_epilogue(0, 0);
-    bool l1_done = false;
     for (uint32_t b = 0; nb_cur != 0u; ++b) {
-      for (int l = l1_done ? 2 : 1; l < 9; ++l) conv_epilogue(b, l);
-      l1_done = false;
+      for (int l = 1; l < 9; ++l) conv_epilogue(b, l);
       head_epilogue(b);
-      if (et == 0) s_nb[4] = mbar_test(bar_batch(b + 1), ((b + 1) >> 1) & 1u) ? s_nb[(b + 1) & 3u] : NOT_YET;
-      epi_bar_sync();
-      uint32_t nb_next = s_nb[4];
-      float w_heads[8][8];
-      if (nb_next != NOT_YET) {
-        load_head_weights(w_heads, 0);
-        if (nb_next != 0u) conv_epilogue(b + 1, 0);
-        if (NOUT <= 8 && nb_next != 0u) {
-          heads_partials(b, w_heads);
-          epi_bar_sync();
-          conv_epilogue(b + 1, 1);
-          l1_done = true;
-          heads_reduce(b, 0);
-          heads_softmax(b);
-        } else {
-          linear_heads(b, w_heads);
-        }
-      } else {
-        load_head_weights(w_heads, 0);
-        linear_heads(b, w_heads);
-        nb_next = wait_batch(b + 1);
-        if (nb_next != 0u) conv_epilogue(b + 1, 0);
-      }
-      nb_cur = nb_next;
-    }
-  }
-
+      nb_cur = wait_batch(b + 1);
+      if (nb_cur != 0u) conv_epilogue(b + 1, 0);
+    }
+  }
   if (RING && warp >= EPI_WARP0 + N_EPI_WARPS) {
     SPB_REGS_TREE();
     tree_worker<G>(T, C, lane);
   } else if (warp == SPARE_WARP) {
     SPB_REGS_LIGHT();
-    const float* s_logits = reinterpret_cast<const float*>(smem + Sm::OFF_LOGITS);
+    const float* s_hpart = reinterpret_cast<const float*>(smem + Sm::OFF_HPART);
+    const float* fcb = reinterpret_cast<const float*>(smem + Sm::OFF_BIAS) + N_LAYERS * 64;
     const uint32_t* s_slots = reinterpret_cast<const uint32_t*>(smem + Sm::OFF_SLOTS);
     for (uint32_t b = 0;; ++b) {
       const uint32_t nb = wait_batch(b);
@@ -761,9 +657,28 @@
       float rec[G::A + 1];
       if ((uint32_t)lane < nb) {
         slot = s_slots[(b & 1u) * Ge::NB + lane];
-#pragma unroll
-        for (int a = 0; a < G::A; ++a) rec[a] = s_logits[lane * 16 + a];
-        rec[G::A] = s_logits[lane * 16 + 15];
+        const float* hp = s_hpart + lane * Sm::HPART_BOARD;
+        float acc[G::A + 1];
+#pragma unroll
+        for (int o = 0; o <= G::A; ++o) acc[o] = hp[o];
+#pragma unroll
+        for (int k = 1; k < 2 * Ge::HG; ++k) {
+#pragma unroll
+          for (int o = 0; o <= G::A; ++o) acc[o] += hp[k * Sm::NOUTP + o];
+        }
+        float mx = -INFINITY;
+#pragma unroll
+        for (int a = 0; a < G::A; ++a) { rec[a] = acc[a] + fcb[a]; mx = fmaxf(mx, rec[a]); }
+        if (logits_out) {
+#pragma unroll
+          for (int a = 0; a < G::A; ++a) logits_out[(size_t)slot * G::A + a] = rec[a];
+        }
+        float sum = 0.0f;
+#pragma unroll
+        for (int a = 0; a < G::A; ++a) { rec[a] = expf(rec[a] - mx); sum += rec[a]; }
+#pragma unroll
+        for (int a = 0; a < G::A; ++a) rec[a] = rec[a] / sum;
+        rec[G::A] = tanhf(acc[G::A] + fcb[16]);
       }
       __syncwarp();
       if (lane == 0) mbar_arrive(bar_out_free);
@@ -847,8 +762,8 @@
 }
 extern "C" int spb_debug_trace_stager(unsigned long long* out) { return (int)cudaMemcpyFromSymbol(out, g_trace_stager, sizeof(unsigned long long) * 16 * 4); }
 extern "C" int spb_debug_trace_v2(unsigned long long* out, int reset) {
-  int rc = (int)cudaMemcpyFromSymbol(out, g_trace, sizeof(unsigned long long) * 4 * 512);
-  if (reset) { static unsigned long long z[4 * 512]; rc |= (int)cudaMemcpyToSymbol(g_trace, z, sizeof z); }
+  int rc = (int)cudaMemcpyFromSymbol(out, g_trace, sizeof(unsigned long long) * 4 * 1024);
+  if (reset) { static unsigned long long z[4 * 1024]; rc |= (int)cudaMemcpyToSymbol(g_trace, z, sizeof z); }
   return rc;
 }
 #endif
diff --git a/self-play-ai_b200/csrc/umma_ptx.cuh b/self-play-ai_b200/csrc/umma_ptx.cuh
--- a/self-play-ai_b200/csrc/umma_ptx.cuh
+++ b/self-play-ai_b200/csrc/umma_ptx.cuh
@@ -38,12 +38,6 @@
     if (NS > 0) __nanosleep(NS);
   }
 }
-__device__ __forceinline__ bool mbar_test(uint32_t bar, uint32_t parity) {
-  uint32_t ok;
-  asm volatile("{\n.reg .pred p;\nmbarrier.test_wait.parity.shared::cta.b64 p, [%1], %2;\nselp.u32 %0, 1, 0, p;\n}"
-               : "=r"(ok) : "r"(bar), "r"(parity) : "memory");
-  return ok != 0;
-}
 __device__ __forceinline__ void mbar_arrive(uint32_t bar) { asm volatile("mbarrier.arrive.shared::cta.b64 _, [%0];" ::"r"(bar) : "memory"); }
 __device__ __forceinline__ void mbar_expect_tx(uint32_t bar, uint32_t bytes) { asm volatile("mbarrier.arrive.expect_tx.shared::cta.b64 _, [%0], %1;" ::"r"(bar), "r"(bytes) : "memory"); }
 __device__ __forceinline__ void bulk_g2s(uint32_t dst, const void* src, uint32_t bytes, uint32_t bar) {
@@ -67,7 +61,6 @@
   asm volatile("{\n.reg .pred P1;\nelect.sync _|P1, 0xffffffff;\nselp.u32 %0, 1, 0, P1;\n}" : "=r"(pred));
   return pred != 0;
 }
-__device__ __forceinline__ void epi_bar_sync() { asm volatile("bar.sync 1, 256;" ::: "memory"); }
 
 __device__ __forceinline__ void tmem_ld16(uint32_t taddr, uint32_t* r) {
   asm volatile("tcgen05.ld.sync.aligned.32x32b.x16.b32 {%0,%1,%2,%3,%4,%5,%6,%7,%8,%9,%10,%11,%12,%13,%14,%15}, [%16];"
@@ -105,6 +98,14 @@
   asm("add.rn.f32x2 %0, %0, %1;" : "+l"(x) : "l"(y));
   asm("mov.b64 {%0, %1}, %2;" : "=f"(x0), "=f"(x1) : "l"(x));
 }
+__device__ __forceinline__ void fma2(float& s0, float& s1, float x0, float x1, float y0, float y1) {
+  uint64_t s, x, y;
+  asm("mov.b64 %0, {%1, %2};" : "=l"(s) : "f"(s0), "f"(s1));
+  asm("mov.b64 %0, {%1, %2};" : "=l"(x) : "f"(x0), "f"(x1));
+  asm("mov.b64 %0, {%1, %2};" : "=l"(y) : "f"(y0), "f"(y1));
+  asm("fma.rn.f32x2 %0, %1, %2, %0;" : "+l"(s) : "l"(x), "l"(y));
+  asm("mov.b64 {%0, %1}, %2;" : "=f"(s0), "=f"(s1) : "l"(s));
+}
 __device__ __forceinline__ uint32_t pack_relu_bf16x2(float lo, float hi) {
   uint32_t d;
   asm("cvt.rn.relu.bf16x2.f32 %0, %1, %2;" : "=r"(d) : "f"(hi), "f"(lo));
```
